# nomic-ai/contrastors

Hardware: AMD Instinct MI355X
Metric: query-doc pairs/sec (whole node), nomic-bert-2048 seq128 global-batch 16384 (higher is better)
Workload: dtype bf16

## Files before the change

contrastors_amd/_C.py:

```python
from __future__ import annotations

import ctypes as C
import os
from pathlib import Path

_PKG = Path(__file__).resolve().parent
LIB_PATH = Path(os.environ.get("CONTRASTORS_HIP_LIB", _PKG / "lib" / "libcontrastors_hip.so"))

CX_OK = 0
_ERR = {-1: "CX_ERR_SHAPE", -2: "CX_ERR_ALIGN", -3: "CX_ERR_ARG", -4: "CX_ERR_LAUNCH"}

vp = C.c_void_p
i32 = C.c_int
i64 = C.c_long
f32 = C.c_float
u64 = C.c_ulonglong
u32 = C.c_uint


class CxLayerWeights(C.Structure):
    _fields_ = (
        [(n, vp) for n in ("Wqkv", "Wout", "Wfc1", "Wfc2", "WqkvT", "WoutT", "Wfc1T", "Wfc2T")]
        + [(n, vp) for n in ("bqkv", "bout", "bfc1", "bfc2")]
        + [(n, vp) for n in ("ln1_g", "ln1_b", "ln2_g", "ln2_b")]
        + [(n, vp) for n in ("gWqkv", "gWout", "gWfc1", "gWfc2")]
        + [(n, vp) for n in ("gbqkv", "gbout", "gbfc1", "gbfc2")]
        + [(n, vp) for n in ("gln1_g", "gln1_b", "gln2_g", "gln2_b")]
    )


class CxEncoderDesc(C.Structure):
    _fields_ = [
        ("n_layer", i32), ("d", i32), ("n_head", i32), ("d_inner", i32), ("gated", i32),
        ("vocab", i32), ("max_pos", i32), ("padding_idx", i32),
        ("ln_eps", f32), ("softmax_scale", f32),
        ("word_emb", vp), ("type_emb", vp), ("pos_emb", vp),
        ("emb_ln_g", vp), ("emb_ln_b", vp),
        ("gword_emb", vp), ("gtype_emb", vp), ("gpos_emb", vp), ("gemb_ln_g", vp), ("gemb_ln_b", vp),
        ("rot_cos", vp), ("rot_sin", vp),
        ("layers", C.POINTER(CxLayerWeights)),
        ("pool_mode", i32), ("normalize", i32),
        ("prenorm", i32),
        ("lnf_g", vp), ("lnf_b", vp), ("glnf_g", vp), ("glnf_b", vp),
        ("Wpatch", vp), ("bpatch", vp), ("cls_token", vp), ("vit_pos", vp),
        ("gWpatch", vp), ("gbpatch", vp), ("gcls_token", vp), ("gvit_pos", vp),
        ("patch_dim", i32),
        ("resid_pdrop", f32), ("embd_pdrop", f32), ("attn_pdrop", f32),
        ("mlp_act", i32), ("lnpre_g", vp), ("lnpre_b", vp), ("glnpre_g", vp), ("glnpre_b", vp),
    ]


class CxChunkBuffers(C.Structure):
    _fields_ = [("T_cap", i64)] + [
        (n, vp)
        for n in (
            "h0", "emb_mean", "emb_rstd", "qkv", "ctx", "lse", "z1", "h1", "mean1", "rstd1", "yg", "act", "z2",
            "h2", "mean2", "rstd2", "pool_norm", "g_a", "g_b", "g_c", "g_wide", "g_act", "tr_a", "tr_b", "delta",
            "ws_f32",
        )
    ] + [("ws_floats", i64)] + [(n, vp) for n in ("zf", "hf", "meanf", "rstdf", "patch_in", "patch_proj")] + [("checkpoint", i32), ("drop_active", i32), ("drop_seed", C.c_ulonglong), ("drop_offset", C.c_ulonglong), ("g_d", vp), ("layer_events", C.POINTER(vp)), ("zpre", vp), ("ckpt_keep", i32), ("patch_keep", vp), ("patch_inv", vp), ("n_keep", i32), ("n_patch_all", i32)]



class CxVitSubLN(C.Structure):
    _fields_ = [(n, vp) for n in ("norm_g", "norm_b", "gnorm_g", "gnorm_b")]


class CxVitExt(C.Structure):
    _fields_ = [("rope_cos", vp), ("rope_sin", vp), ("n_rope", i32), ("n_prefix", i32), ("no_final_ln", i32),
                ("subln_eps", f32), ("sub_ln", C.POINTER(CxVitSubLN)), ("z", vp), ("zmean", vp), ("zrstd", vp),
                ("yg_wide", vp)]


_SIGS = {
    "cx_abi_version": (i32, []),
    "cx_build_info": (C.c_char_p, []),
    "cx_error_string": (C.c_char_p, [i32]),
    "cx_gemm_bf16_nt": (i32, [vp, vp, vp, vp, i32, i32, i32, i32, i32, i32, i32, i32, f32, vp]),
    "cx_gemm_bf16_nt_accum": (i32, [vp, vp, vp, vp, i64, i32, i32, i32, i32, i32, vp]),
    "cx_gemm_bf16_tn_accum": (i32, [vp, vp, vp, vp, i64, i32, i32, i32, i32, i32, vp]),
    "cx_prof_gemm_config": (i32, [i32, i32]),
    "cx_prof_gemm_collect": (i32, [C.POINTER(C.c_double), C.POINTER(C.c_double), C.POINTER(i64), C.POINTER(i64)]),
    "cx_calib_mfma_bf16": (i32, [vp, i32, i32, vp, vp, vp]),
    "cx_calib_copy": (i32, [vp, vp, i64, vp]),
    "cx_transpose_bf16": (i32, [vp, vp, i32, i32, i32, i32, i32, vp]),
    "cx_cast_f32_to_bf16": (i32, [vp, vp, i64, vp]),
    "cx_cast_transpose_f32_to_bf16": (i32, [vp, vp, i32, i32, vp]),
    "cx_cast_transpose_f32_to_bf16_batched": (i32, [vp, i32, i32, vp]),
    "cx_cast_bf16_to_f32": (i32, [vp, vp, i64, vp]),
    "cx_layernorm_fwd": (i32, [vp, vp, vp, vp, vp, vp, vp, vp, i32, i32, f32, vp]),
    "cx_layernorm_bwd": (i32, [vp, vp, vp, vp, vp, vp, vp, vp, vp, vp, vp, i64, i32, i32, vp]),
    "cx_layernorm_bwd_pooled": (i32, [vp, vp, vp, vp, i32, i32, i32, vp, vp, vp, vp, vp, vp, vp, vp, vp, i64, i32, i32, vp]),
    "cx_layernorm_bwd_colsum": (i32, [vp, vp, vp, vp, vp, vp, vp, vp, vp, vp, vp, vp, i64, i32, i32, vp]),
    "cx_dropout_add_layernorm_fwd": (i32, [vp, vp, vp, vp, vp, vp, vp, vp, i32, i32, f32, f32, C.c_ulonglong, C.c_ulonglong,
                                           C.c_uint, vp]),
    "cx_dropout_add_layernorm_bwd": (i32, [vp, vp, vp, vp, vp, vp, vp, vp, vp, vp, vp, i64, i32, i32, f32, C.c_ulonglong,
                                           C.c_ulonglong, C.c_uint, vp]),
    "cx_dropout_add_layernorm_bwd_colsum": (i32, [vp, vp, vp, vp, vp, vp, vp, vp, vp, vp, vp, vp, i64, i32, i32, f32, C.c_ulonglong,
                                                  C.c_ulonglong, C.c_uint, vp]),
    "cx_dropout_scale": (i32, [vp, i64, f32, C.c_ulonglong, C.c_ulonglong, C.c_uint, vp]),
    "cx_layernorm_fwd_mixed": (i32, [vp, vp, vp, vp, vp, vp, vp, vp, i32, i32, f32, i32, vp]),
    "cx_layernorm_bwd_mixed": (i32, [vp, vp, vp, vp, vp, vp, vp, vp, vp, vp, i32, i32, i32, vp]),
    "cx_embed_ln_fwd": (i32, [vp, vp, vp, vp, vp, vp, vp, vp, vp, vp, i32, i32, i32, f32, vp]),
    "cx_embed_ln_bwd": (i32, [vp] * 15 + [i32, i32, i32, i32, vp]),
    "cx_embed_ln_bwd_sorted": (i32, [vp] * 15 + [i32, i32, i32, i32, i32, vp, vp, vp, vp]),
    "cx_swiglu_fwd": (i32, [vp, vp, i32, i32, i32, vp]),
    "cx_swiglu_bwd": (i32, [vp, vp, vp, i32, i32, i32, vp]),
    "cx_gemm_bf16_swiglu": (i32, [vp, vp, vp, vp, i32, i32, i32, i32, i32, i32, i32, vp]),
    "cx_gemm_bf16_nt_residual": (i32, [vp, vp, vp, vp, vp, i32, i32, i32, i32, i32, i32, i32, vp]),
    "cx_gemm_bf16_swiglu_bwd": (i32, [vp, vp, vp, vp, i32, i32, i32, i32, i32, i32, vp]),
    "cx_gemm_bf16_nt_splitk": (i32, [vp, vp, vp, vp, vp, vp, i64, i32, i32, i32, i32, i32, i32, i32, vp]),
    "cx_gemm_bf16_swiglu_gate": (i32, [vp, vp, vp, vp, i32, i32, i32, i32, i32, i32, i32, vp]),
    "cx_gemm_bf16_swiglu_bwd_gate": (i32, [vp, vp, vp, vp, vp, i32, i32, i32, i32, i32, i32, i32, vp]),
    "cx_swiglu_bwd_gate": (i32, [vp, vp, vp, vp, i32, i32, vp]),
    "cx_gemm_bf16_bias_gelu": (i32, [vp, vp, vp, vp, vp, i32, i32, i32, i32, i32, i32, i32, vp]),
    "cx_gemm_bf16_bias_act": (i32, [vp, vp, vp, vp, vp, i32, i32, i32, i32, i32, i32, i32, i32, vp]),
    "cx_bias_gelu_fwd": (i32, [vp, vp, vp, i32, i32, vp]),
    "cx_bias_gelu_bwd": (i32, [vp, vp, vp, vp, i32, i32, vp]),
    "cx_bias_grad": (i32, [vp, vp, i32, i32, i32, vp]),
    "cx_bias_gelu_bwd_colsum": (i32, [vp, vp, vp, vp, vp, i32, i32, vp]),
    "cx_bias_act_fwd": (i32, [vp, vp, vp, i32, i32, i32, vp]),
    "cx_bias_act_bwd_colsum": (i32, [vp, vp, vp, vp, vp, i32, i32, i32, vp]),
    "cx_gemm_bf16_act_bwd": (i32, [vp, vp, vp, vp, vp, vp, i64, i32, i32, i32, i32, i32, i32, i32, i32, vp]),
    "cx_attn_varlen_fwd": (i32, [vp, vp, vp, vp, vp, vp, i32, i32, i32, i32, f32, vp]),
    "cx_attn_varlen_bwd": (i32, [vp] * 9 + [i32, i32, i32, i32, f32, vp]),
    "cx_attn_varlen_bwd_prerotated": (i32, [vp] * 9 + [i32, i32, i32, i32, f32, vp]),
    "cx_attn_varlen_dropout_fwd": (i32, [vp] * 6 + [i32, i32, i32, i32, f32, f32, u64, u64, u32, vp]),
    "cx_attn_varlen_dropout_bwd": (i32, [vp] * 9 + [i32, i32, i32, i32, f32, f32, u64, u64, u32, vp]),
    "cx_ipc_alloc": (i32, [C.POINTER(vp), i64, i32]),
    "cx_ipc_free": (i32, [vp]),
    "cx_ipc_export": (i32, [vp, vp]),
    "cx_ipc_open": (i32, [vp, C.POINTER(vp)]),
    "cx_ipc_close": (i32, [vp]),
    "cx_xgmi_push": (i32, [vp, vp, i64, i64, i32, vp]),
    "cx_xgmi_scatter": (i32, [vp, vp, i32, i64, i32, vp]),
    "cx_xgmi_signal_wait": (i32, [vp, vp, i32, i32, u32, i64, vp, vp]),
    "cx_sum_slots_f32": (i32, [vp, vp, i64, i32, vp]),
    "cx_attn_varlen_kvpacked_fwd": (i32, [vp] * 6 + [i32, i32, i32, i32, i32, f32, vp]),
    "cx_attn_varlen_kvpacked_bwd": (i32, [vp] * 10 + [i32, i32, i32, i32, i32, f32, vp]),
    "cx_rotary_qkv_inplace": (i32, [vp, vp, vp, vp, i32, i32, i32, i32, i32, vp]),
    "cx_rotary_apply": (i32, [vp, i64, vp, vp, vp, i32, i32, i32, i32, i32, vp]),
    "cx_pool_normalize_fwd": (i32, [vp, vp, vp, vp, i32, i32, i32, i32, vp]),
    "cx_pool_normalize_bwd": (i32, [vp, vp, vp, vp, vp, i32, i32, i32, i32, vp]),
    "cx_vit_patchify": (i32, [vp, i32, vp, i32, i32, i32, i32, i32, vp]),
    "cx_vit_assemble_fwd": (i32, [vp, vp, vp, vp, i32, i32, i32, vp]),
    "cx_vit_assemble_bwd": (i32, [vp, vp, vp, vp, i32, i32, i32, vp]),
    "cx_vit_patchify_gather": (i32, [vp, i32, vp, i32, i32, i32, i32, i32, vp, i32, vp]),
    "cx_vit_assemble_fwd_gather": (i32, [vp, vp, vp, vp, i32, i32, i32, vp, vp]),
    "cx_vit_assemble_bwd_gather": (i32, [vp, vp, vp, vp, i32, i32, i32, vp, i32, vp]),
    "cx_vit_forward": (i32, [C.POINTER(CxEncoderDesc), C.POINTER(CxChunkBuffers), vp, i32, vp, i32, i32, i32, i32, i32,
                             i32, vp, vp]),
    "cx_vit_backward": (i32, [C.POINTER(CxEncoderDesc), C.POINTER(CxChunkBuffers), vp, i32, i32, vp, vp, vp]),
    "cx_vit_forward_hidden": (i32, [C.POINTER(CxEncoderDesc), C.POINTER(CxChunkBuffers), vp, i32, vp, i32, i32, i32, i32, i32,
                                    i32, vp, vp]),
    "cx_vit_backward_hidden": (i32, [C.POINTER(CxEncoderDesc), C.POINTER(CxChunkBuffers), vp, i32, i32, vp, vp]),
    "cx_rope2d_qkv_inplace": (i32, [vp, vp, vp, vp, i32, i32, i32, i32, i32, i32, vp]),
    "cx_swiglu_subln_fwd": (i32, [vp, vp, vp, vp, vp, vp, vp, vp, i32, i32, f32, vp]),
    "cx_swiglu_subln_bwd": (i32, [vp] * 11 + [i64, i32, i32, vp]),
    "cx_vit_forward_ex": (i32, [C.POINTER(CxEncoderDesc), C.POINTER(CxChunkBuffers), C.POINTER(CxVitExt), vp, i32, vp, i32, i32,
                                i32, i32, i32, i32, vp, vp]),
    "cx_vit_backward_ex": (i32, [C.POINTER(CxEncoderDesc), C.POINTER(CxChunkBuffers), C.POINTER(CxVitExt), vp, i32, i32, vp, vp,
                                 vp]),
# ... 150 lines not shown
```

contrastors_amd/config.py:

```python
from __future__ import annotations

from typing import Any, Dict, List, Optional, Tuple, Union

import yaml
from pydantic import BaseModel, ConfigDict, model_validator


class TrainArgs(BaseModel):
    model_config = ConfigDict(extra="ignore", validate_assignment=True)
    num_epochs: int = 1
    num_train_steps: Optional[int] = None
    learning_rate: float = 2e-4
    weight_decay: float = 0.01
    eps: Optional[float] = 1e-8
    warmup_steps: Optional[int] = None
    warmup_pct: Optional[float] = None
    cooldown_steps: Optional[int] = None
    checkpoint: Optional[str] = None
    wandb: bool = False
    wandb_project_name: str = ""
    wandb_entity: str = ""
    wandb_run_name: Optional[str] = None
    wandb_group: Optional[str] = None
    log_grads_every: int = 100
    log_lr_every: int = 10
    save_every: Optional[int] = None
    eval_steps: Optional[int] = None
    eval_strategy: Optional[str] = None
    output_dir: Optional[str] = None
    gradient_accumulation_steps: Optional[int] = 1
    schedule_type: str = "cosine"
    max_grad_norm: float = 1.0
    adam_beta1: float = 0.9
    adam_beta2: float = 0.999
    loss_fn: Optional[str] = "clip"
    grad_cache: Optional[bool] = None
    chunk_size: Optional[int] = None
    clamp_logits: Optional[bool] = True
    logit_max: Optional[float] = 100.0
    matryoshka_dims: Optional[List[int]] = None
    matryoshka_loss_weights: Optional[List[float]] = None
    profile: Optional[bool] = False
    use_fp8: Optional[bool] = False
    gradcache_chunk: Union[int, str, None] = "auto"
    gradcache_resident: Union[bool, str, None] = "auto"
    exchange: Optional[str] = "auto"
    exchange_timeout_s: float = 120.0
    overlap_grad_reduce: bool = True
    checkpoint_keep_layers: Union[int, str, None] = "auto"
    distill_loss_fn: str = "mse"
    distill_temperature: float = 1.0

    @model_validator(mode="after")
    def _checks(self):
        from .policy import _parse_chunk, _parse_keep, _parse_resident

        _parse_chunk(self.gradcache_chunk, "train_args.gradcache_chunk")
        _parse_resident(self.gradcache_resident, "train_args.gradcache_resident")
        _parse_keep(self.checkpoint_keep_layers, "train_args.checkpoint_keep_layers")
        if self.distill_loss_fn not in ("mse", "kd", "towers", "stella"):
            raise ValueError(f"Loss function {self.distill_loss_fn} not found in loss function registry")
        if self.exchange not in (None, "auto", "rccl", "oneshot"):
            raise ValueError(f"train_args.exchange must be auto, rccl or oneshot, got {self.exchange!r}")
        if self.use_fp8 and self.matryoshka_dims is not None:
            bad = [d for d in self.matryoshka_dims if d not in (256, 512, 768, 1024)]
            if bad:
                raise ValueError(f"use_fp8 covers similarity widths 256 / 512 / 768 / 1024; matryoshka_dims has {bad}")
        if self.eval_strategy is not None and self.eval_strategy not in ("steps", "epochs"):
            raise ValueError(f"Eval strategy {self.eval_strategy} not found in eval strategy registry")
        if self.eval_strategy == "steps" and self.eval_steps is None:
            raise ValueError("Eval steps must be set if eval strategy is set to steps")
        if self.matryoshka_dims is not None and self.grad_cache:
            raise ValueError("Matryoshka dims cannot be set if grad cache is set")
        return self


class DataArgs(BaseModel):
    model_config = ConfigDict(extra="ignore")
    shuffle: bool = False
    workers: int = 0
    batch_size: int = 16384
    seed: int = 42
    input_shards: Optional[str] = None
    download: Optional[bool] = False
    streaming: Optional[bool] = True
    process_one_shard: Optional[bool] = False
    weighted_sampling: Optional[bool] = False
    verbose: Optional[bool] = False
    sample_negatives: Optional[bool] = False
    query_max_length: Optional[int] = None
    document_max_length: Optional[int] = None
    mlm_prob: Optional[float] = None
    tokenized_dataset: Optional[str] = None
    val_pct: Optional[float] = None
    val_mlm_prob: Optional[float] = None
    mask_on: str = "device"
    task_name: Optional[str] = None
    image_text_shards: Optional[str] = None
# ... 102 lines not shown
```

contrastors_amd/csrc/engine.hip:

```cpp
#include <hip/hip_runtime.h>
#include "../../include/contrastors_hip.h"
#include "ln_workspace.h"

namespace {

#define CX_TRY(expr)              \
    do {                          \
        int rc__ = (expr);        \
        if (rc__ != CX_OK) return rc__; \
    } while (0)

inline long round_up(long v, long m) { return (v + m - 1) / m * m; }

inline int mark_grads_done(const CxChunkBuffers* buf, int idx, void* stream) {
    if (!buf->layer_events || !buf->layer_events[idx]) return CX_OK;
    return hipEventRecord((hipEvent_t)buf->layer_events[idx], (hipStream_t)stream) == hipSuccess ? CX_OK : CX_ERR_LAUNCH;
}

struct Slots {
    const CxChunkBuffers* b;
    const CxEncoderDesc* e;
    long T_cap;
    int d, I, wfc1;
    int mode;
    int first_kept;
    bool kept(int s) const { return mode == 1 || (mode == 2 && s >= first_kept); }
    int sl(int s) const { return mode == 1 ? s : (mode == 2 && s >= first_kept) ? 1 + s - first_kept : 0; }
    int sl_in(int s) const { return mode == 0 ? 0 : s; }
    uint16_t* qkv(int s) const { return b->qkv + (size_t)sl(s) * T_cap * 3 * d; }
    uint16_t* ctx(int s) const { return b->ctx + (size_t)sl(s) * T_cap * d; }
    float* lse(int s) const { return b->lse + (size_t)sl(s) * T_cap * e->n_head; }
    uint16_t* z1(int s) const { return b->z1 + (size_t)(e->prenorm ? sl_in(s) : sl(s)) * T_cap * d; }
    uint16_t* h1(int s) const { return b->h1 + (size_t)sl(s) * T_cap * d; }
    float* mean1(int s) const { return b->mean1 + (size_t)sl(s) * T_cap; }
    float* rstd1(int s) const { return b->rstd1 + (size_t)sl(s) * T_cap; }
    uint16_t* yg(int s) const { return b->yg + (size_t)sl(s) * T_cap * I; }
    uint16_t* act(int s) const { return b->act + (size_t)sl(s) * T_cap * I; }
    uint16_t* z2(int s) const { return b->z2 + (size_t)sl(s) * T_cap * d; }
    uint16_t* h2(int s) const { return b->h2 + (size_t)(e->prenorm ? sl(s) : sl_in(s)) * T_cap * d; }
    float* mean2(int s) const { return b->mean2 + (size_t)sl(s) * T_cap; }
    float* rstd2(int s) const { return b->rstd2 + (size_t)sl(s) * T_cap; }
    uint16_t* ez(const CxVitExt* x, int s) const { return x->z + (size_t)sl(s) * T_cap * I; }
    float* ezmean(const CxVitExt* x, int s) const { return x->zmean + (size_t)sl(s) * T_cap; }
    float* ezrstd(const CxVitExt* x, int s) const { return x->zrstd + (size_t)sl(s) * T_cap; }
};

inline bool ext_rope(const CxVitExt* x) { return x && x->rope_cos; }
inline bool ext_subln(const CxVitExt* x) { return x && x->sub_ln; }
inline bool ext_no_lnf(const CxVitExt* x) { return x && x->no_final_ln; }
int check_ext(const CxVitExt* x, const CxEncoderDesc* e, const CxChunkBuffers* b) {
    if (!x) return CX_OK;
    if (x->rope_cos && (!x->rope_sin || x->n_rope <= 0 || x->n_prefix < 0)) return CX_ERR_ARG;
    if (x->sub_ln) {
        if (!e->gated || !x->z || !x->zmean || !x->zrstd || (!x->yg_wide && !b->g_wide)) return CX_ERR_ARG;
        for (int l = 0; l < e->n_layer; ++l)
            if (!x->sub_ln[l].norm_g || !x->sub_ln[l].norm_b) return CX_ERR_ARG;
    }
    return CX_OK;
}

Slots make_slots(const CxEncoderDesc* enc, const CxChunkBuffers* buf, int save) {
    const int L = enc->n_layer;
    int keep = buf->ckpt_keep < 0 ? 0 : buf->ckpt_keep > L ? L : buf->ckpt_keep;
    return Slots{buf, enc, buf->T_cap, enc->d, enc->d_inner, enc->gated ? 2 * enc->d_inner : enc->d_inner,
                 save ? (buf->checkpoint ? 2 : 1) : 0, L - keep};
}

int check_desc(const CxEncoderDesc* e, const CxChunkBuffers* b, int T) {
    if (!e || !b || !e->layers) return CX_ERR_ARG;
    if (e->n_layer <= 0 || e->d <= 0 || e->n_head <= 0) return CX_ERR_ARG;
    if (e->d != e->n_head * 64) return CX_ERR_SHAPE;
    if ((e->d % 64) != 0 || (e->d_inner % 64) != 0) return CX_ERR_SHAPE;
    if (b->T_cap < round_up(T, 64)) return CX_ERR_SHAPE;
    return CX_OK;
}

int wgrad_split(int out_f, int in_f, long Tp) {
    const long tiles = (long)((out_f + 127) / 128) * ((in_f + 127) / 128);
    const long nk = Tp / 64;
    long s = (512 + tiles - 1) / tiles;
    if (s > nk / 2) s = nk / 2;
    if (s < 1) s = 1;
    return (int)s;
}

int wgrad(const uint16_t* dY, int out_f, const uint16_t* X, int in_f, float* gW, const CxChunkBuffers* b, int T,
          void* stream) {
    if (!gW) return CX_OK;
    const int rc = cx_gemm_bf16_tn_accum(dY, X, gW, b->ws_f32, b->ws_floats, T, out_f, in_f, out_f, in_f, stream);
    if (rc != CX_ERR_SHAPE) return rc;
    if (!b->tr_a || !b->tr_b) return CX_ERR_ARG;
    const int Tp = (int)round_up(T, 64);
    CX_TRY(cx_transpose_bf16(dY, b->tr_a, T, out_f, out_f, Tp, Tp, stream));
    CX_TRY(cx_transpose_bf16(X, b->tr_b, T, in_f, in_f, Tp, Tp, stream));
    return cx_gemm_bf16_nt_accum(b->tr_a, b->tr_b, gW, b->ws_f32, b->ws_floats, out_f, in_f, Tp, Tp, Tp, stream);
}

int proj_residual(const uint16_t* x, const uint16_t* W, const float* bias, const uint16_t* residual, uint16_t* out, int T,
                  int N, int K, bool* folded, void* stream, const CxChunkBuffers* buf = nullptr) {
    *folded = false;
    if (buf && buf->ws_f32 && (long)((T + 255) / 256) * ((N + 255) / 256) <= 64 && K >= 1536) {
        const int rc = cx_gemm_bf16_nt_splitk(x, W, out, bias, residual, buf->ws_f32, buf->ws_floats, T, N, K, K, K, N, N, stream);
        if (rc != CX_ERR_SHAPE) {
            *folded = residual != nullptr && rc == CX_OK;
            return rc;
        }
    }
    if (residual) {
        const int rc = cx_gemm_bf16_nt_residual(x, W, out, bias, residual, T, N, K, K, K, N, N, stream);
        if (rc != CX_ERR_SHAPE) {
            *folded = rc == CX_OK;
            return rc;
        }
    }
    return cx_gemm_bf16_nt(x, W, out, bias, T, N, K, K, K, N, 0, 1, 1.f, stream);
}

bool gelu_fused_shape(int T, int N, int K) {
    return T > 0 && (K % 64) == 0 && (N % 8) == 0;
}

struct BlockRunner {
    const CxEncoderDesc* enc;
    const CxChunkBuffers* buf;
    const Slots& s;
    const int32_t* cu_seqlens;
    int Bc, T, max_seqlen;
    void* stream;
    const CxVitExt* ext = nullptr;

    int mlp_up(const CxLayerWeights& w, const uint16_t* x, int l, bool keep) const {
        const int d = enc->d, I = enc->d_inner;
        if (ext_subln(ext)) {
            uint16_t* yg = ext->yg_wide ? ext->yg_wide : buf->g_wide;
            CX_TRY(cx_gemm_bf16_nt(x, w.Wfc1, yg, w.bfc1, T, 2 * I, d, d, d, 2 * I, 0, 1, 1.f, stream));
            const CxVitSubLN& n = ext->sub_ln[l];
            return cx_swiglu_subln_fwd(yg, n.norm_g, n.norm_b, keep ? s.yg(l) : nullptr, s.act(l), s.ez(ext, l), s.ezmean(ext, l),
                                       s.ezrstd(ext, l), T, I, ext->subln_eps, stream);
        }
        if (enc->gated) {
            return cx_gemm_bf16_swiglu_gate(x, w.Wfc1, keep ? s.yg(l) : nullptr, s.act(l), T, I, d, d, d, I, I, stream);
        }
        const int rc = cx_gemm_bf16_bias_act(x, w.Wfc1, w.bfc1, keep ? s.yg(l) : nullptr, s.act(l), T, s.wfc1, d, d, d, s.wfc1,
                                             I, enc->mlp_act, stream);
        if (rc != CX_ERR_SHAPE) return rc;
        CX_TRY(cx_gemm_bf16_nt(x, w.Wfc1, s.yg(l), nullptr, T, s.wfc1, d, d, d, s.wfc1, 0, 1, 1.f, stream));
        return cx_bias_act_fwd(s.yg(l), w.bfc1, s.act(l), T, I, enc->mlp_act, stream);
    }
    int mlp(const CxLayerWeights& w, const uint16_t* x, int l, uint16_t* out, const uint16_t* residual, bool keep,
            bool* folded) const {
        CX_TRY(mlp_up(w, x, l, keep));
        return proj_residual(ext_subln(ext) ? s.ez(ext, l) : s.act(l), w.Wfc2, w.bfc2, residual, out, T, enc->d, enc->d_inner, folded, stream, buf);
    }
    int attn(const CxLayerWeights& w, const uint16_t* x, int l, uint16_t* out, const uint16_t* residual, bool* folded) const {
        const int d = enc->d;
        CX_TRY(cx_gemm_bf16_nt(x, w.Wqkv, s.qkv(l), w.bqkv, T, 3 * d, d, d, d, 3 * d, 0, 1, 1.f, stream));
        if (ext_rope(ext))
            CX_TRY(cx_rope2d_qkv_inplace(s.qkv(l), cu_seqlens, ext->rope_cos, ext->rope_sin, ext->n_rope, Bc, enc->n_head, T,
                                         ext->n_prefix, 1, stream));
        if (buf->drop_active && enc->attn_pdrop > 0.f) {
            CX_TRY(cx_attn_varlen_dropout_fwd(s.qkv(l), cu_seqlens, enc->rot_cos, enc->rot_sin, s.ctx(l), s.lse(l), Bc,
                                              enc->n_head, T, max_seqlen, enc->softmax_scale, enc->attn_pdrop, buf->drop_seed,
                                              buf->drop_offset, (unsigned)(2 * enc->n_layer + 1 + l), stream));
        } else if (enc->rot_cos && max_seqlen > 128) {
            CX_TRY(cx_rotary_qkv_inplace(s.qkv(l), cu_seqlens, enc->rot_cos, enc->rot_sin, Bc, enc->n_head, T, max_seqlen, 1,
                                         stream));
            CX_TRY(cx_attn_varlen_fwd(s.qkv(l), cu_seqlens, nullptr, nullptr, s.ctx(l), s.lse(l), Bc, enc->n_head, T, max_seqlen,
                                      enc->softmax_scale, stream));
        } else {
            CX_TRY(cx_attn_varlen_fwd(s.qkv(l), cu_seqlens, enc->rot_cos, enc->rot_sin, s.ctx(l), s.lse(l), Bc, enc->n_head, T,
                                      max_seqlen, enc->softmax_scale, stream));
        }
        return proj_residual(s.ctx(l), w.Wout, w.bout, residual, out, T, d, d, folded, stream);
    }
    int post_block(int l, const uint16_t* h_in, bool keep) const {
        const CxLayerWeights& w = enc->layers[l];
        const int d = enc->d;
        bool f1 = false, f2 = false;
        if (drop()) {
            const float p = enc->resid_pdrop;
            CX_TRY(attn(w, h_in, l, s.z1(l), nullptr, &f1));
            CX_TRY(cx_dropout_add_layernorm_fwd(s.z1(l), h_in, w.ln1_g, w.ln1_b, s.h1(l), keep ? s.z1(l) : nullptr, s.mean1(l),
                                                s.rstd1(l), T, d, enc->ln_eps, p, buf->drop_seed, buf->drop_offset, 2 * l, stream));
            CX_TRY(mlp(w, s.h1(l), l, s.z2(l), nullptr, keep, &f2));
            return cx_dropout_add_layernorm_fwd(s.z2(l), s.h1(l), w.ln2_g, w.ln2_b, s.h2(l), keep ? s.z2(l) : nullptr, s.mean2(l),
                                                s.rstd2(l), T, d, enc->ln_eps, p, buf->drop_seed, buf->drop_offset, 2 * l + 1,
                                                stream);
        }
        CX_TRY(attn(w, h_in, l, s.z1(l), h_in, &f1));
        CX_TRY(cx_layernorm_fwd(s.z1(l), f1 ? nullptr : h_in, w.ln1_g, w.ln1_b, s.h1(l), (keep && !f1) ? s.z1(l) : nullptr,
                                s.mean1(l), s.rstd1(l), T, d, enc->ln_eps, stream));
        CX_TRY(mlp(w, s.h1(l), l, s.z2(l), s.h1(l), keep, &f2));
        return cx_layernorm_fwd(s.z2(l), f2 ? nullptr : s.h1(l), w.ln2_g, w.ln2_b, s.h2(l), (keep && !f2) ? s.z2(l) : nullptr,
                                s.mean2(l), s.rstd2(l), T, d, enc->ln_eps, stream);
    }
    bool drop() const { return buf->drop_active && enc->resid_pdrop > 0.f; }
    int pre_block(int l, const uint16_t* x, const uint16_t* r, bool r_folded, bool keep, bool up_only, const uint16_t** x_out,
                  const uint16_t** r_out, bool* folded_out) const {
        const CxLayerWeights& w = enc->layers[l];
        const int d = enc->d, L = enc->n_layer;
        CX_TRY(cx_layernorm_fwd(x, r, w.ln1_g, w.ln1_b, s.h1(l), (r_folded && x == s.z1(l)) ? nullptr : s.z1(l), s.mean1(l),
                                s.rstd1(l), T, d, enc->ln_eps, stream));
        bool f1 = false, f2 = false;
        CX_TRY(attn(w, s.h1(l), l, s.z2(l), s.z1(l), &f1));
        CX_TRY(cx_layernorm_fwd(s.z2(l), f1 ? nullptr : s.z1(l), w.ln2_g, w.ln2_b, s.h2(l), f1 ? nullptr : s.z2(l), s.mean2(l),
                                s.rstd2(l), T, d, enc->ln_eps, stream));
        if (up_only) return mlp_up(w, s.h2(l), l, keep);
        uint16_t* nxt = (l + 1 < L) ? s.z1(l + 1) : buf->zf;
        CX_TRY(mlp(w, s.h2(l), l, nxt, s.z2(l), keep, &f2));
        *x_out = nxt;
        *r_out = f2 ? nullptr : s.z2(l);
        *folded_out = f2;
        return CX_OK;
    }
};

int blocks_forward(const CxEncoderDesc* enc, const CxChunkBuffers* buf, const Slots& s, const uint16_t* h0,
                   const int32_t* cu_seqlens, int Bc, int T, int max_seqlen, int save, const uint16_t** h_final,
                   void* stream, const CxVitExt* ext = nullptr) {
    const int d = enc->d, L = enc->n_layer;
    const BlockRunner run{enc, buf, s, cu_seqlens, Bc, T, max_seqlen, stream, ext};
    if (!enc->prenorm) {
        const uint16_t* h_in = h0;
        for (int l = 0; l < L; ++l) {
            CX_TRY(run.post_block(l, h_in, save != 0 && s.kept(l)));
            h_in = s.h2(l);
        }
        *h_final = h_in;
        return CX_OK;
    }
    if (!buf->zf || !buf->hf || !buf->meanf || !buf->rstdf || (!ext_no_lnf(ext) && (!enc->lnf_g || !enc->lnf_b))) return CX_ERR_ARG;
    if (buf->drop_active && enc->resid_pdrop > 0.f) return CX_ERR_ARG;
    const uint16_t* x = h0;
    const uint16_t* r = nullptr;
    bool r_folded = false;
    for (int l = 0; l < L; ++l) {
        CX_TRY(run.pre_block(l, x, r, r_folded, save != 0 && s.kept(l), false, &x, &r, &r_folded));
        if (save == 2 && !r_folded) return CX_ERR_SHAPE;
    }
    if (ext_no_lnf(ext)) {
        if (!r_folded || x != buf->zf) return CX_ERR_SHAPE;
        *h_final = buf->zf;
        return CX_OK;
    }
    CX_TRY(cx_layernorm_fwd(x, r, enc->lnf_g, enc->lnf_b, buf->hf, r_folded ? nullptr : buf->zf, buf->meanf, buf->rstdf, T,
// ... 533 lines not shown
```

contrastors_amd/csrc/gemm_api.hip:

```cpp
#include "cx_common.h"
#include "../../include/contrastors_hip.h"
#include "gemm_params.h"
#include <mutex>

namespace {

constexpr int BK = 64;

__global__ __launch_bounds__(256) void splitk_reduce_kernel(const float* __restrict__ part, float* __restrict__ out, long n4,
                                                            long slab, int splits) {
    const long stride = (long)gridDim.x * blockDim.x;
    for (long i = (long)blockIdx.x * blockDim.x + threadIdx.x; i < n4; i += stride) {
        float4 a = reinterpret_cast<const float4*>(out)[i];
        for (int s = 0; s < splits; ++s) {
            const float4 v = reinterpret_cast<const float4*>(part + s * slab)[i];
            a.x += v.x; a.y += v.y; a.z += v.z; a.w += v.w;
        }
        reinterpret_cast<float4*>(out)[i] = a;
    }
}

int reduce_slabs(const float* ws, float* out, long slab, int split, hipStream_t s) {
    const long n4 = slab / 4;
    long g = (n4 + 255) / 256;
// ... 113 lines not shown
    const int Tp = (T + BK - 1) / BK * BK;
    GemmParams p = base_params(dY, A, ws, nullptr, O, I, Tp, ld_dy, ld_a, I);
    const long tiles = (long)(O / 256) * (I / 256), nk = Tp / BK;
    long max_split = nk / 4;
    if (max_split > ws_floats / slab) max_split = ws_floats / slab;
    if (max_split > 32) max_split = 32;
    p.split_k = (int)choose_split(tiles, max_split);
    {
        ProfScope prof(2.0 * (double)T * (double)O * (double)I, (hipStream_t)stream);
        if (cx_launch_gemm_v6_tn(p, (hipStream_t)stream) != hipSuccess) return CX_ERR_LAUNCH;
    }
    return reduce_slabs(ws, G, slab, p.split_k, (hipStream_t)stream);
}

int cx_gemm_bf16_swiglu(const uint16_t* X, const uint16_t* W, uint16_t* YG, uint16_t* Act, int M, int I, int K, int ldx,
                        int ldw, int ld_yg, int ld_act, void* stream) {
    if (M <= 0 || I <= 0) return CX_OK;
    if (K <= 0 || (K % BK) != 0 || (I % 32) != 0) return CX_ERR_SHAPE;
    if ((ldx % 8) != 0 || (ldw % 8) != 0 || (ld_yg % 4) != 0 || (ld_act % 4) != 0) return CX_ERR_ALIGN;
    if (!Act) return CX_ERR_ARG;
    GemmParams p = base_params(X, W, YG, nullptr, M, 2 * I, K, ldx, ldw, ld_yg);
    p.Out2 = Act; p.ldo2 = ld_act;
    ProfScope prof(2.0 * (double)M * (double)(2 * I) * (double)K, (hipStream_t)stream);
    const hipError_t e = ((ld_yg % 8) == 0 && (ld_act % 8) == 0)
                             ? cx_launch_gemm_v6(p, GEMM_EPI_SWIGLU, (hipStream_t)stream)
                             : cx_launch_gemm_v5(p, 0, GEMM_OUT_BF16, GEMM_EPI_SWIGLU, (hipStream_t)stream);
    return e == hipSuccess ? CX_OK : CX_ERR_LAUNCH;
}

int cx_gemm_bf16_swiglu_gate(const uint16_t* X, const uint16_t* W, uint16_t* G, uint16_t* Act, int M, int I, int K, int ldx,
                             int ldw, int ld_g, int ld_act, void* stream) {
    if (M <= 0 || I <= 0) return CX_OK;
    if (K <= 0 || (K % BK) != 0 || (I % 32) != 0 || (ld_g % 8) != 0 || (ld_act % 8) != 0) return CX_ERR_SHAPE;
    if ((ldx % 8) != 0 || (ldw % 8) != 0) return CX_ERR_ALIGN;
    if (!Act) return CX_ERR_ARG;
    GemmParams p = base_params(X, W, G, nullptr, M, 2 * I, K, ldx, ldw, ld_g);
    p.Out2 = Act; p.ldo2 = ld_act;
    ProfScope prof(2.0 * (double)M * (double)(2 * I) * (double)K, (hipStream_t)stream);
    return cx_launch_gemm_v6(p, GEMM_EPI_SWIGLU_G, (hipStream_t)stream) == hipSuccess ? CX_OK : CX_ERR_LAUNCH;
}

int cx_gemm_bf16_nt_residual(const uint16_t* X, const uint16_t* W, uint16_t* Out, const float* bias, const uint16_t* Residual,
                             int M, int N, int K, int ldx, int ldw, int ldo, int ldr, void* stream) {
    if (M <= 0 || N <= 0) return CX_OK;
    if (!Residual || !Out) return CX_ERR_ARG;
    if (K <= 0 || (K % 64) != 0 || (N % 8) != 0 || (ldo % 8) != 0 || (ldr % 8) != 0) return CX_ERR_SHAPE;
    if ((ldx % 8) != 0 || (ldw % 8) != 0) return CX_ERR_ALIGN;
    GemmParams p = base_params(X, W, Out, bias, M, N, K, ldx, ldw, ldo);
    p.Out2 = const_cast<uint16_t*>(Residual); p.ldo2 = ldr;
    ProfScope prof(2.0 * (double)M * (double)N * (double)K, (hipStream_t)stream);
    return cx_launch_gemm_v6(p, GEMM_EPI_NONE, (hipStream_t)stream) == hipSuccess ? CX_OK : CX_ERR_LAUNCH;
}

int cx_gemm_bf16_bias_gelu(const uint16_t* X, const uint16_t* W, const float* bias, uint16_t* Pre, uint16_t* Act, int M, int N,
                           int K, int ldx, int ldw, int ld_pre, int ld_act, void* stream) {
    return cx_gemm_bf16_bias_act(X, W, bias, Pre, Act, M, N, K, ldx, ldw, ld_pre, ld_act, 0, stream);
}

int cx_gemm_bf16_bias_act(const uint16_t* X, const uint16_t* W, const float* bias, uint16_t* Pre, uint16_t* Act, int M, int N,
                          int K, int ldx, int ldw, int ld_pre, int ld_act, int act, void* stream) {
    if (M <= 0 || N <= 0) return CX_OK;
    if (!Act || (act != 0 && act != 1)) return CX_ERR_ARG;
    if (K <= 0 || (K % 64) != 0 || (N % 8) != 0 || (ld_act % 8) != 0 || (Pre && (ld_pre % 8) != 0)) return CX_ERR_SHAPE;
    if ((ldx % 8) != 0 || (ldw % 8) != 0) return CX_ERR_ALIGN;
    GemmParams p = base_params(X, W, Pre, bias, M, N, K, ldx, ldw, ld_pre);
    p.Out2 = Act; p.ldo2 = ld_act;
    p.act = act;
    ProfScope prof(2.0 * (double)M * (double)N * (double)K, (hipStream_t)stream);
    return cx_launch_gemm_v6(p, act == 1 ? GEMM_EPI_QGELU : GEMM_EPI_GELU, (hipStream_t)stream) == hipSuccess ? CX_OK : CX_ERR_LAUNCH;
}

int cx_gemm_bf16_swiglu_bwd(const uint16_t* dY, const uint16_t* W, const uint16_t* YG, uint16_t* dYG, int M, int I, int K,
                            int ldx, int ldw, int ld_yg, void* stream) {
    if (M <= 0 || I <= 0) return CX_OK;
    if (!dY || !W || !YG || !dYG) return CX_ERR_ARG;
    if (K <= 0 || (K % 64) != 0 || (I % 256) != 0 || (ld_yg % 8) != 0 || ld_yg < 2 * I) return CX_ERR_SHAPE;
    if ((ldx % 8) != 0 || (ldw % 8) != 0) return CX_ERR_ALIGN;
    GemmParams p = base_params(dY, W, dYG, nullptr, M, I, K, ldx, ldw, ld_yg);
    p.Out2 = const_cast<uint16_t*>(YG); p.ldo2 = ld_yg;
    ProfScope prof(2.0 * (double)M * (double)I * (double)K, (hipStream_t)stream);
    return cx_launch_gemm_v6(p, GEMM_EPI_SWIGLU_BWD, (hipStream_t)stream) == hipSuccess ? CX_OK : CX_ERR_LAUNCH;
}

int cx_gemm_bf16_swiglu_bwd_gate(const uint16_t* dY, const uint16_t* W, const uint16_t* Act, const uint16_t* G, uint16_t* dYG,
                                 int M, int I, int K, int ldx, int ldw, int ld_ag, int ld_dyg, void* stream) {
    if (M <= 0 || I <= 0) return CX_OK;
    if (!dY || !W || !Act || !G || !dYG) return CX_ERR_ARG;
    if (K <= 0 || (K % 64) != 0 || (I % 256) != 0 || (ld_dyg % 8) != 0 || ld_dyg < 2 * I || (ld_ag % 8) != 0 || ld_ag < I)
        return CX_ERR_SHAPE;
    if ((ldx % 8) != 0 || (ldw % 8) != 0) return CX_ERR_ALIGN;
    GemmParams p = base_params(dY, W, dYG, nullptr, M, I, K, ldx, ldw, ld_dyg);
    p.Out2 = const_cast<uint16_t*>(Act); p.ldo2 = ld_ag;
    p.In3 = G;
    ProfScope prof(2.0 * (double)M * (double)I * (double)K, (hipStream_t)stream);
    return cx_launch_gemm_v6(p, GEMM_EPI_SWIGLU_BWD_AG, (hipStream_t)stream) == hipSuccess ? CX_OK : CX_ERR_LAUNCH;
}

int cx_gemm_bf16_act_bwd(const uint16_t* dY, const uint16_t* W, const uint16_t* Pre, uint16_t* dPre, float* dbias, float* ws,
                         long ws_floats, int M, int N, int K, int ldx, int ldw, int ld_pre, int ld_dpre, int act, void* stream) {
    if (M <= 0 || N <= 0) return CX_OK;
    if (!dY || !W || !Pre || !dPre || (act != 0 && act != 1)) return CX_ERR_ARG;
    if (K <= 0 || (K % 64) != 0 || (N % 8) != 0 || (ld_pre % 8) != 0 || (ld_dpre % 8) != 0) return CX_ERR_SHAPE;
    if ((ldx % 8) != 0 || (ldw % 8) != 0) return CX_ERR_ALIGN;
    const int nblocks = (M + 127) / 128;
    if (dbias && (!ws || ws_floats < (long)nblocks * N)) return CX_ERR_SHAPE;
    GemmParams p = base_params(dY, W, dPre, nullptr, M, N, K, ldx, ldw, ld_dpre);
// ... 41 lines not shown
```

contrastors_amd/csrc/gemm_bf16.hip:

```cpp
#include "cx_common.h"
#include "../../include/contrastors_hip.h"
#include "gemm_params.h"

namespace {

constexpr int BM = 128, BN = 128, BK = 64;
constexpr int TILE_BYTES = 128 * BK * 2;

typedef __attribute__((address_space(3))) void* lds_void_ptr;
typedef const __attribute__((address_space(1))) void* glb_void_ptr;

enum OutMode { OUT_BF16 = GEMM_OUT_BF16, OUT_F32 = GEMM_OUT_F32, OUT_F32_ATOMIC = GEMM_OUT_F32_ATOMIC };

struct StageRegs { uint4 r0, r1, r2, r3; };

CX_DEVICE uint4 stage_load(const bf16_t* __restrict__ base, int ld, int row0, int nrows, int k0, int tid, int p) {
    const int r = p * 32 + (tid >> 3);
    int gr = row0 + r;
    gr = gr < nrows ? gr : nrows - 1;
    return *reinterpret_cast<const uint4*>(base + (size_t)gr * ld + k0 + (tid & 7) * 8);
}

template <bool GLDS>
CX_DEVICE void stage_tile(const bf16_t* __restrict__ base, int ld, int row0, int nrows, int k0, char* lds_tile,
// ... 745 lines not shown
    p.tiles_m = p.tiles_n = 0; p.split_k = 1; p.alpha = 1.f; p.dbg = g_dbg;
    p.Out2 = Act; p.ldo2 = ld_act; p.sup_m = p.sup_n = 0;
    int slot = -1;
    if (g_prof.enabled) {
        if ((g_prof.launches % g_prof.stride) == 0 && g_prof.used < GemmProf::CAP) {
            slot = g_prof.used++;
            if (slot >= g_prof.created) {
                if (hipEventCreate(&g_prof.ev0[slot]) != hipSuccess || hipEventCreate(&g_prof.ev1[slot]) != hipSuccess)
                    return CX_ERR_LAUNCH;
                g_prof.created = slot + 1;
            }
            g_prof.flop[slot] = 2.0 * (double)M * (double)(2 * I) * (double)K;
            (void)hipEventRecord(g_prof.ev0[slot], (hipStream_t)stream);
        }
        ++g_prof.launches;
    }
    hipError_t e = cx_launch_gemm_v5(p, 0, GEMM_OUT_BF16, GEMM_EPI_SWIGLU, (hipStream_t)stream);
    if (slot >= 0) (void)hipEventRecord(g_prof.ev1[slot], (hipStream_t)stream);
    return e == hipSuccess ? CX_OK : CX_ERR_LAUNCH;
}

int cx_gemm_bf16_nt_residual(const uint16_t* X, const uint16_t* W, uint16_t* Out, const float* bias,
                             const uint16_t* Residual, int M, int N, int K, int ldx, int ldw, int ldo, int ldr,
                             void* stream) {
    if (M <= 0 || N <= 0) return CX_OK;
    if (!Residual || !Out) return CX_ERR_ARG;
    if (K <= 0 || (K % 64) != 0 || (N % 8) != 0 || (ldo % 8) != 0 || (ldr % 8) != 0) return CX_ERR_SHAPE;
    if ((ldx % 8) != 0 || (ldw % 8) != 0) return CX_ERR_ALIGN;
    if (cx_gemm_get_variant() != 6) return CX_ERR_SHAPE;
    GemmParams p;
    p.X = X; p.W = W; p.Out = Out; p.bias = bias;
    p.M = M; p.N = N; p.K = K; p.ldx = ldx; p.ldw = ldw; p.ldo = ldo;
    p.tiles_m = p.tiles_n = 0; p.split_k = 1; p.alpha = 1.f; p.dbg = g_dbg;
    p.Out2 = const_cast<uint16_t*>(Residual); p.ldo2 = ldr; p.sup_m = p.sup_n = 0; p.trace = nullptr;
    int slot = -1;
    if (g_prof.enabled) {
        if ((g_prof.launches % g_prof.stride) == 0 && g_prof.used < GemmProf::CAP) {
            slot = g_prof.used++;
            if (slot >= g_prof.created) {
                if (hipEventCreate(&g_prof.ev0[slot]) != hipSuccess || hipEventCreate(&g_prof.ev1[slot]) != hipSuccess)
                    return CX_ERR_LAUNCH;
                g_prof.created = slot + 1;
            }
            g_prof.flop[slot] = 2.0 * (double)M * (double)N * (double)K;
            (void)hipEventRecord(g_prof.ev0[slot], (hipStream_t)stream);
        }
        ++g_prof.launches;
    }
    const hipError_t e = cx_launch_gemm_v6(p, GEMM_EPI_NONE, (hipStream_t)stream);
    if (slot >= 0) (void)hipEventRecord(g_prof.ev1[slot], (hipStream_t)stream);
    return e == hipSuccess ? CX_OK : CX_ERR_LAUNCH;
}

int cx_gemm_bf16_bias_gelu(const uint16_t* X, const uint16_t* W, const float* bias, uint16_t* Pre, uint16_t* Act, int M,
                           int N, int K, int ldx, int ldw, int ld_pre, int ld_act, void* stream) {
    return cx_gemm_bf16_bias_act(X, W, bias, Pre, Act, M, N, K, ldx, ldw, ld_pre, ld_act, 0, stream);
}

int cx_gemm_bf16_bias_act(const uint16_t* X, const uint16_t* W, const float* bias, uint16_t* Pre, uint16_t* Act, int M,
                          int N, int K, int ldx, int ldw, int ld_pre, int ld_act, int act, void* stream) {
    if (M <= 0 || N <= 0) return CX_OK;
    if (!Act || (act != 0 && act != 1)) return CX_ERR_ARG;
    if (K <= 0 || (K % 64) != 0 || (N % 8) != 0 || (ld_act % 8) != 0 || (Pre && (ld_pre % 8) != 0)) return CX_ERR_SHAPE;
    if ((ldx % 8) != 0 || (ldw % 8) != 0) return CX_ERR_ALIGN;
    if (cx_gemm_get_variant() != 6) return CX_ERR_SHAPE;
    GemmParams p;
    p.X = X; p.W = W; p.Out = Pre; p.bias = bias;
    p.M = M; p.N = N; p.K = K; p.ldx = ldx; p.ldw = ldw; p.ldo = ld_pre;
    p.tiles_m = p.tiles_n = 0; p.split_k = 1; p.alpha = 1.f; p.dbg = g_dbg;
    p.Out2 = Act; p.ldo2 = ld_act; p.sup_m = p.sup_n = 0; p.trace = nullptr;
    p.act = act;
    int slot = -1;
    if (g_prof.enabled) {
        if ((g_prof.launches % g_prof.stride) == 0 && g_prof.used < GemmProf::CAP) {
            slot = g_prof.used++;
            if (slot >= g_prof.created) {
                if (hipEventCreate(&g_prof.ev0[slot]) != hipSuccess || hipEventCreate(&g_prof.ev1[slot]) != hipSuccess)
                    return CX_ERR_LAUNCH;
                g_prof.created = slot + 1;
            }
            g_prof.flop[slot] = 2.0 * (double)M * (double)N * (double)K;
            (void)hipEventRecord(g_prof.ev0[slot], (hipStream_t)stream);
        }
        ++g_prof.launches;
    }
    const hipError_t e = cx_launch_gemm_v6(p, act == 1 ? GEMM_EPI_QGELU : GEMM_EPI_GELU, (hipStream_t)stream);
    if (slot >= 0) (void)hipEventRecord(g_prof.ev1[slot], (hipStream_t)stream);
    return e == hipSuccess ? CX_OK : CX_ERR_LAUNCH;
}

int cx_gemm_bf16_swiglu_bwd(const uint16_t* dY, const uint16_t* W, const uint16_t* YG, uint16_t* dYG, int M, int I, int K,
                            int ldx, int ldw, int ld_yg, void* stream) {
    if (M <= 0 || I <= 0) return CX_OK;
    if (!dY || !W || !YG || !dYG) return CX_ERR_ARG;
    if (K <= 0 || (K % 64) != 0 || (I % 256) != 0 || (ld_yg % 8) != 0 || ld_yg < 2 * I) return CX_ERR_SHAPE;
    if ((ldx % 8) != 0 || (ldw % 8) != 0) return CX_ERR_ALIGN;
    if (cx_gemm_get_variant() != 6) return CX_ERR_SHAPE;
    GemmParams p;
    p.X = dY; p.W = W; p.Out = dYG; p.bias = nullptr;
    p.M = M; p.N = I; p.K = K; p.ldx = ldx; p.ldw = ldw; p.ldo = ld_yg;
    p.tiles_m = p.tiles_n = 0; p.split_k = 1; p.alpha = 1.f; p.dbg = g_dbg;
    p.Out2 = const_cast<uint16_t*>(YG); p.ldo2 = ld_yg; p.sup_m = p.sup_n = 0; p.trace = nullptr;
    int slot = -1;
    if (g_prof.enabled) {
        if ((g_prof.launches % g_prof.stride) == 0 && g_prof.used < GemmProf::CAP) {
            slot = g_prof.used++;
// ... 92 lines not shown
```

contrastors_amd/csrc/gemm_bf16_v6.hip:

```cpp
#include "cx_common.h"
#include "../../include/contrastors_hip.h"
#include "gemm_params.h"
#include <type_traits>

namespace {

#ifndef CX_V6_HI_EARLY
#define CX_V6_HI_EARLY 1
#endif
#ifndef CX_V6_OPAQUE
#define CX_V6_OPAQUE 1
#endif
#ifndef CX_V6_NT
#define CX_V6_NT 3
#endif
template <int J>
__device__ __forceinline__ void v6_dma_m0(uint32_t slot_base) {
    asm volatile("s_add_u32 m0, %0, %1" ::"s"(slot_base), "n"(J * 4096) : "memory", "scc");
}
__device__ __forceinline__ void v6_dma_ld(uint32_t off, const bf16_t* base) {
    asm volatile("global_load_lds_dwordx4 %0, %1" ::"v"(off), "s"(base) : "memory");
}
template <int J>
__device__ __forceinline__ void v6_dma_full(uint32_t slot_base, uint32_t off, const bf16_t* base) {
    asm volatile("s_add_u32 m0, %0, %1\n\ts_nop 0\n\tglobal_load_lds_dwordx4 %2, %3" ::"s"(slot_base), "n"(J * 4096), "v"(off),
                 "s"(base) : "memory", "scc");
}
typedef unsigned int cx_u32x4 __attribute__((ext_vector_type(4)));
__device__ __forceinline__ void gst_nt(void* ptr, uint4 v) {
    cx_u32x4 t = {v.x, v.y, v.z, v.w};
    __builtin_nontemporal_store(t, reinterpret_cast<cx_u32x4*>(ptr));
}
__device__ __forceinline__ uint4 gld_nt(const void* ptr) {
    const cx_u32x4 t = __builtin_nontemporal_load(reinterpret_cast<const cx_u32x4*>(ptr));
    return make_uint4(t.x, t.y, t.z, t.w);
}
#if CX_V6_NT & 1
#define gst(ptr, v) gst_nt((ptr), (v))
#else
#define gst(ptr, v) (*reinterpret_cast<uint4*>(ptr) = (v))
#endif
#if CX_V6_NT & 2
#define gld(ptr) gld_nt(ptr)
#else
#define gld(ptr) (*reinterpret_cast<const uint4*>(ptr))
#endif

typedef __attribute__((address_space(3))) void* lds_void_ptr;
typedef const __attribute__((address_space(1))) void* glb_void_ptr;

constexpr int BM6 = 256, BN6 = 256, BK6 = 64;
constexpr int XS6 = 32768;
constexpr int LDS6 = 5 * XS6;

struct Frags6 {
// ... 201 lines not shown
        const char* xs = dsm + xs_slot * XS6;
        const char* ws = dsm + (3 + ws_slot) * XS6;
        const int nxs_slot = xs_slot == 2 ? 0 : xs_slot + 1, nws_slot = ws_slot ^ 1;
        if constexpr (decltype(first)::value) {
            CX_SEG(mma1z, F0, 0, 64, F1, xs, ws, 1, RS_ == 2 ? 0 : 1, RS_, 1, RS_ == 2 ? 1 : 17, DS_, 0, 8);
        } else {
            CX_SEG(mma1, F0, 0, 64, F1, xs, ws, 1, RS_ == 2 ? 0 : 1, RS_, 1, RS_ == 2 ? 1 : 17, DS_, 0, 8);
        }
        w_advance();
        CX_SEG(mma1, F1, 0, 32, F0, xs, ws, 0, 0, 0, 2, 0, RS_ == 2 ? 8 : DS_, 0, 4);
        asm volatile("s_waitcnt lgkmcnt(0)" ::: "memory");
        if constexpr ((DBG & 128) != 0) {
            const long long w0_ = (long long)__builtin_amdgcn_s_memtime();
            asm volatile("s_waitcnt vmcnt(4)" ::: "memory");
            const long long w1_ = (long long)__builtin_amdgcn_s_memtime();
            ph[decltype(first)::value ? 0 : 1] += w1_ - w0_;
        } else if constexpr ((DBG & 32) == 0) {
            asm volatile("s_waitcnt vmcnt(4)" ::: "memory");
        }
        if constexpr ((DBG & 2) == 0) __builtin_amdgcn_s_barrier();
        const char* nxs = dsm + nxs_slot * XS6;
        const char* nws = dsm + (3 + nws_slot) * XS6;
        CX_SEG(mma1, F1, 32, 64, F0, nxs, nws, 0, RS_ == 2 ? 32 : 33, RS_, 2, RS_ == 2 ? 33 : 49, RS_ == 2 ? 8 : DS_, 4, 4);
        x_advance();
        if constexpr ((DBG & 128) != 0 && decltype(first)::value) {
            const long long now_ = (long long)__builtin_amdgcn_s_memtime();
            kt0_cyc += now_ - t_last;
        }
        ++cp_kt;
        pxs_slot = xs_slot;
        pws_slot = ws_slot;
        xs_slot = nxs_slot;
        ws_slot = nws_slot;
    };

#pragma unroll 1
    while (cp_tile >= 0) {
        cp_kt = 0;
        kt_body(std::true_type{});
#pragma unroll 1
        while (cp_kt < nk) kt_body(std::false_type{});

        {
            CX_PH(2);
            asm volatile("s_nop 7\n\ts_nop 7\n\ts_nop 7" ::: "memory");
            const int tn = cp_tile & 255, tm = cp_tile >> 8;
            const int m0 = tm * BM6 + wm * 128, n0 = tn * BN6 + wn * 128;
            char* my = ((wave < 2) ? dsm + pxs_slot * XS6 : dsm + (3 + pws_slot) * XS6) + (wave & 1) * 16384;
            constexpr int ROWB = 272;
            auto prow = [&](int q) { return (q >> 1) * 16 + l15; };
            auto pcol = [&](int q) { return (q & 1) * 16 + 4 * g4; };
            auto qoff = [](int q, int rowb) { return (q >> 1) * 16 * rowb + (q & 1) * 32; };
            if constexpr ((DBG & 16) != 0) {
            } else if constexpr (EPI == GEMM_EPI_NONE || EPI == GEMM_EPI_ACT_BWD || EPI == GEMM_EPI_QACT_BWD) {
                constexpr bool ACTB = EPI == GEMM_EPI_ACT_BWD || EPI == GEMM_EPI_QACT_BWD;
                float cs0 = 0.f, cs1 = 0.f, cs2 = 0.f, cs3 = 0.f, cs4 = 0.f, cs5 = 0.f, cs6 = 0.f, cs7 = 0.f;
                constexpr int act_kind = EPI == GEMM_EPI_QACT_BWD ? CX_ACT_QUICK_GELU : CX_ACT_GELU;
                auto mul_grad = [&](uint4& v, const uint4& r) {
#define CX_MG(w_, ca, cb)                                                                              \
    {                                                                                                 \
        const float o0 = bf16lo_to_f32(v.w_) * act_grad(bf16lo_to_f32(r.w_), act_kind);               \
        const float o1 = bf16hi_to_f32(v.w_) * act_grad(bf16hi_to_f32(r.w_), act_kind);               \
        v.w_ = pack_bf16x2(o0, o1);                                                                   \
        ca += bf16lo_to_f32(v.w_);                                                                    \
        cb += bf16hi_to_f32(v.w_);                                                                    \
    }
                    CX_MG(x, cs0, cs1) CX_MG(y, cs2, cs3) CX_MG(z, cs4, cs5) CX_MG(w, cs6, cs7)
#undef CX_MG
                };
                auto flush_colsum = [&]() {
                    if constexpr (ACTB) {
                        float c[8] = {cs0, cs1, cs2, cs3, cs4, cs5, cs6, cs7};
#pragma unroll
                        for (int e = 0; e < 8; ++e) {
                            c[e] += __shfl_xor(c[e], 16, 64);
                            c[e] += __shfl_xor(c[e], 32, 64);
                        }
                        const int n = n0 + (lane & 15) * 8;
                        if (p.colsum_part && lane < 16 && m0 < p.M && n + 8 <= p.N) {
                            float* dst = p.colsum_part + (size_t)(m0 >> 7) * p.N + n;
                            *reinterpret_cast<float4*>(dst) = make_float4(c[0], c[1], c[2], c[3]);
                            *reinterpret_cast<float4*>(dst + 4) = make_float4(c[4], c[5], c[6], c[7]);
                        }
                    }
                };
                const bool add_bias = p.bias != nullptr;
                const bf16_t* resid = reinterpret_cast<const bf16_t*>(p.Out2);
                auto fast_tile = [&](auto with_resid) {
                    constexpr bool RES = decltype(with_resid)::value;
                    const int rrow = lane >> 4, rch = lane & 15;
                    bf16_t* outp = reinterpret_cast<bf16_t*>(p.Out) + (size_t)(m0 + rrow) * p.ldo + n0 + rch * 8;
                    const bf16_t* resp = RES ? resid + (size_t)(m0 + rrow) * p.ldo2 + n0 + rch * 8 : nullptr;
                    const char* rd = my + rrow * ROWB + rch * 16;
                    char* wr = my + prow(0) * ROWB + pcol(0) * 2;
                    uint2 pk[16];
                    auto pack_pass = [&](int b) {
#pragma unroll
                        for (int a = 0; a < 4; ++a) {
                            float blk[16];
                            v6_read_block(4 * b + a, blk);
#pragma unroll
                            for (int q = 0; q < 4; ++q) {
                                pk[a * 4 + q].x = pack_bf16x2(blk[4 * q], blk[4 * q + 1]);
                                pk[a * 4 + q].y = pack_bf16x2(blk[4 * q + 2], blk[4 * q + 3]);
                            }
                        }
                    };
                    auto stage = [&]() {
#pragma unroll
                        for (int a = 0; a < 4; ++a)
#pragma unroll
                            for (int q = 0; q < 4; ++q) *reinterpret_cast<uint2*>(wr + a * 64 + qoff(q, ROWB)) = pk[a * 4 + q];
                    };
                    uint4 r0 = {}, r1 = {}, r2 = {}, r3 = {}, r4 = {}, r5 = {}, r6 = {}, r7 = {};
#define CX_RES_ROWS(b_)                                                                                   \
    r0 = gld(resp + (size_t)((b_) * 32 + 0) * p.ldo2);                          \
    r1 = gld(resp + (size_t)((b_) * 32 + 4) * p.ldo2);                          \
    r2 = gld(resp + (size_t)((b_) * 32 + 8) * p.ldo2);                          \
    r3 = gld(resp + (size_t)((b_) * 32 + 12) * p.ldo2);                         \
    r4 = gld(resp + (size_t)((b_) * 32 + 16) * p.ldo2);                         \
    r5 = gld(resp + (size_t)((b_) * 32 + 20) * p.ldo2);                         \
    r6 = gld(resp + (size_t)((b_) * 32 + 24) * p.ldo2);                         \
    r7 = gld(resp + (size_t)((b_) * 32 + 28) * p.ldo2);
                    auto add_res = [&](uint4& v, const uint4& r) {
                        v.x = pack_bf16x2(bf16lo_to_f32(v.x) + bf16lo_to_f32(r.x), bf16hi_to_f32(v.x) + bf16hi_to_f32(r.x));
                        v.y = pack_bf16x2(bf16lo_to_f32(v.y) + bf16lo_to_f32(r.y), bf16hi_to_f32(v.y) + bf16hi_to_f32(r.y));
                        v.z = pack_bf16x2(bf16lo_to_f32(v.z) + bf16lo_to_f32(r.z), bf16hi_to_f32(v.z) + bf16hi_to_f32(r.z));
                        v.w = pack_bf16x2(bf16lo_to_f32(v.w) + bf16lo_to_f32(r.w), bf16hi_to_f32(v.w) + bf16hi_to_f32(r.w));
                    };
                    auto one_pass = [&](auto bc) {
                        constexpr int b = decltype(bc)::value;
                        uint4 v0 = *reinterpret_cast<const uint4*>(rd + 0 * ROWB), v1 = *reinterpret_cast<const uint4*>(rd + 4 * ROWB),
                              v2 = *reinterpret_cast<const uint4*>(rd + 8 * ROWB), v3 = *reinterpret_cast<const uint4*>(rd + 12 * ROWB),
                              v4 = *reinterpret_cast<const uint4*>(rd + 16 * ROWB), v5 = *reinterpret_cast<const uint4*>(rd + 20 * ROWB),
                              v6 = *reinterpret_cast<const uint4*>(rd + 24 * ROWB), v7 = *reinterpret_cast<const uint4*>(rd + 28 * ROWB);
                        __builtin_amdgcn_sched_barrier(0);
                        if constexpr (b < 3) pack_pass(b + 1);
                        __builtin_amdgcn_sched_barrier(0);
                        if constexpr (RES) {
                            add_res(v0, r0); add_res(v1, r1); add_res(v2, r2); add_res(v3, r3);
                            add_res(v4, r4); add_res(v5, r5); add_res(v6, r6); add_res(v7, r7);
                            if constexpr (b < 3) {
                                __builtin_amdgcn_sched_barrier(0);
                                CX_RES_ROWS(b + 1)
                                __builtin_amdgcn_sched_barrier(0);
                            }
                        }
                        if constexpr (b < 3) stage();
                        bf16_t* o = outp + (size_t)(b * 32) * p.ldo;
                        if constexpr ((DBG & 64) != 0) {
                            const uint4 vs[8] = {v0, v1, v2, v3, v4, v5, v6, v7};
#pragma unroll
                            for (int i = 0; i < 8; ++i) asm volatile("" ::"v"(vs[i].x), "v"(vs[i].y), "v"(vs[i].z), "v"(vs[i].w));
                            asm volatile("" ::"v"(o));
                            return;
                        }
                        gst(o, v0);
                        gst(o + (size_t)4 * p.ldo, v1);
                        gst(o + (size_t)8 * p.ldo, v2);
                        gst(o + (size_t)12 * p.ldo, v3);
                        gst(o + (size_t)16 * p.ldo, v4);
                        gst(o + (size_t)20 * p.ldo, v5);
                        gst(o + (size_t)24 * p.ldo, v6);
                        gst(o + (size_t)28 * p.ldo, v7);
                    };
                    if constexpr (RES) { CX_RES_ROWS(0) }
                    pack_pass(0);
                    stage();
                    one_pass(std::integral_constant<int, 0>{});
                    one_pass(std::integral_constant<int, 1>{});
                    one_pass(std::integral_constant<int, 2>{});
                    one_pass(std::integral_constant<int, 3>{});
#undef CX_RES_ROWS
                };
                auto fast_tile_actb = [&]() {
                    const int rrow = lane >> 4, rch = lane & 15;
                    bf16_t* outp = reinterpret_cast<bf16_t*>(p.Out) + (size_t)(m0 + rrow) * p.ldo + n0 + rch * 8;
                    const bf16_t* resp = resid + (size_t)(m0 + rrow) * p.ldo2 + n0 + rch * 8;
                    const char* rd = my + rrow * ROWB + rch * 16;
                    char* wr = my + prow(0) * ROWB + pcol(0) * 2;
                    auto stage_pass = [&](int b) {
#pragma unroll
                        for (int a = 0; a < 4; ++a) {
                            float blk[16];
                            v6_read_block(4 * b + a, blk);
#pragma unroll
                            for (int q = 0; q < 4; ++q) {
                                uint2 pk2;
                                pk2.x = pack_bf16x2(blk[4 * q], blk[4 * q + 1]);
                                pk2.y = pack_bf16x2(blk[4 * q + 2], blk[4 * q + 3]);
                                *reinterpret_cast<uint2*>(wr + a * 64 + qoff(q, ROWB)) = pk2;
                            }
                            __builtin_amdgcn_sched_barrier(0);
                        }
                    };
                    uint4 r0, r1, r2, r3;
#define CX_PRE_ROWS(hh_)                                                        \
    r0 = gld(resp + (size_t)((hh_) * 16 + 0) * p.ldo2);                         \
    r1 = gld(resp + (size_t)((hh_) * 16 + 4) * p.ldo2);                         \
    r2 = gld(resp + (size_t)((hh_) * 16 + 8) * p.ldo2);                         \
    r3 = gld(resp + (size_t)((hh_) * 16 + 12) * p.ldo2);
                    auto half_pass = [&](auto hc) {
                        constexpr int hh = decltype(hc)::value;
                        constexpr int h = hh & 1;
                        uint4 v0 = *reinterpret_cast<const uint4*>(rd + (h * 16 + 0) * ROWB), v1 = *reinterpret_cast<const uint4*>(rd + (h * 16 + 4) * ROWB),
                              v2 = *reinterpret_cast<const uint4*>(rd + (h * 16 + 8) * ROWB), v3 = *reinterpret_cast<const uint4*>(rd + (h * 16 + 12) * ROWB);
                        __builtin_amdgcn_sched_barrier(0);
                        mul_grad(v0, r0); __builtin_amdgcn_sched_barrier(0);
                        mul_grad(v1, r1); __builtin_amdgcn_sched_barrier(0);
                        mul_grad(v2, r2); __builtin_amdgcn_sched_barrier(0);
                        mul_grad(v3, r3); __builtin_amdgcn_sched_barrier(0);
                        if constexpr (hh < 7) { CX_PRE_ROWS(hh + 1) }
                        __builtin_amdgcn_sched_barrier(0);
                        bf16_t* o = outp + (size_t)(hh * 16) * p.ldo;
                        gst(o, v0);
                        gst(o + (size_t)4 * p.ldo, v1);
                        gst(o + (size_t)8 * p.ldo, v2);
// ... 25 lines not shown
                            CX_RES_LOAD(0, r0) CX_RES_LOAD(1, r1) CX_RES_LOAD(2, r2) CX_RES_LOAD(3, r3)
                            CX_RES_LOAD(4, r4) CX_RES_LOAD(5, r5) CX_RES_LOAD(6, r6) CX_RES_LOAD(7, r7)
#undef CX_RES_LOAD
                        }
#pragma unroll
                        for (int a = 0; a < 4; ++a) {
                            float blk[16];
                            v6_read_block(4 * b + a, blk);
#pragma unroll
                            for (int q = 0; q < 4; ++q) {
                                const int nl = a * 32 + pcol(q);
                                float v[4];
#pragma unroll
                                for (int e = 0; e < 4; ++e) v[e] = blk[4 * q + e];
                                if constexpr (!decltype(plain)::value) {
#pragma unroll
                                    for (int e = 0; e < 4; ++e) v[e] *= p.alpha;
                                    if (add_bias) {
                                        const int n = n0 + nl;
                                        if (n < p.N) {
                                            const float4 bv = *reinterpret_cast<const float4*>(p.bias + n);
                                            v[0] += bv.x; v[1] += bv.y; v[2] += bv.z; v[3] += bv.w;
                                        }
                                    }
                                }
                                uint2 pk;
                                pk.x = pack_bf16x2(v[0], v[1]);
                                pk.y = pack_bf16x2(v[2], v[3]);
                                *reinterpret_cast<uint2*>(my + prow(q) * ROWB + nl * 2) = pk;
                            }
                        }
#pragma unroll
                        for (int ps = 0; ps < 8; ++ps) {
                            const int row = ps * 4 + (lane >> 4), ch = lane & 15;
                            const int m = m0 + b * 32 + row, n = n0 + ch * 8;
                            uint4 vv = *reinterpret_cast<const uint4*>(my + row * ROWB + ch * 16);
                            if (resid && ACTB) {
                                const uint4 rr = ps == 0 ? r0 : ps == 1 ? r1 : ps == 2 ? r2 : ps == 3 ? r3 : ps == 4 ? r4 : ps == 5 ? r5
                                                 : ps == 6 ? r6 : r7;
                                if (m < p.M && n + 8 <= p.N) mul_grad(vv, rr);
                            } else if (resid) {
                                const uint4 rr = ps == 0 ? r0 : ps == 1 ? r1 : ps == 2 ? r2 : ps == 3 ? r3 : ps == 4 ? r4 : ps == 5 ? r5
                                                 : ps == 6 ? r6 : r7;
                                vv.x = pack_bf16x2(bf16lo_to_f32(vv.x) + bf16lo_to_f32(rr.x), bf16hi_to_f32(vv.x) + bf16hi_to_f32(rr.x));
                                vv.y = pack_bf16x2(bf16lo_to_f32(vv.y) + bf16lo_to_f32(rr.y), bf16hi_to_f32(vv.y) + bf16hi_to_f32(rr.y));
                                vv.z = pack_bf16x2(bf16lo_to_f32(vv.z) + bf16lo_to_f32(rr.z), bf16hi_to_f32(vv.z) + bf16hi_to_f32(rr.z));
                                vv.w = pack_bf16x2(bf16lo_to_f32(vv.w) + bf16lo_to_f32(rr.w), bf16hi_to_f32(vv.w) + bf16hi_to_f32(rr.w));
                            }
                            if (m < p.M && n + 8 <= p.N)
                                gst(reinterpret_cast<bf16_t*>(p.Out) + (size_t)m * p.ldo + n, vv);
                        }
                    }
                };
                if constexpr (ACTB) {
                    if (fast) {
                        fast_tile_actb();
                    } else {
                        store_tile(std::true_type{});
                    }
                    flush_colsum();
                } else if (fast) {
                    if (resid) {
                        fast_tile(std::true_type{});
                    } else {
                        fast_tile(std::false_type{});
                    }
                } else if (p.alpha == 1.f && !add_bias) {
                    store_tile(std::true_type{});
                } else {
                    store_tile(std::false_type{});
                }
            } else if constexpr (IS_SWIGLU_BWD) {
                const bf16_t* yg_in = reinterpret_cast<const bf16_t*>(p.Out2);
                const bf16_t* g_in = reinterpret_cast<const bf16_t*>(p.In3);
                bf16_t* dyg = reinterpret_cast<bf16_t*>(p.Out);
                const int c0 = 2 * n0;
                auto bwd_elem = [&](float yv, float gv, float dv, float& dyo, float& dgo) {
                    if constexpr (AG) {
                        swiglu_bwd_from_act(dv, yv, gv, dyo, dgo);
                    } else {
                        const float sg = __builtin_amdgcn_rcpf(1.f + __builtin_amdgcn_exp2f(-1.4426950408889634f * gv));
                        const float gs = gv * sg;
                        dyo = gs * dv;
                        dgo = (sg + gs * (1.f - sg)) * dv * yv;
                    }
                };
                auto bwd_quad = [&](const float (&yv)[4], const float (&gv)[4], const float* dv, float (&dyo)[4], float (&dgo)[4]) {
                    if constexpr (AG) {
#pragma unroll
                        for (int h = 0; h < 2; ++h) {
                            cx_f2 y2, g2;
                            swiglu_bwd_from_act2(cx_f2{dv[2 * h], dv[2 * h + 1]}, cx_f2{yv[2 * h], yv[2 * h + 1]},
                                                 cx_f2{gv[2 * h], gv[2 * h + 1]}, y2, g2);
                            dyo[2 * h] = y2.x; dyo[2 * h + 1] = y2.y;
                            dgo[2 * h] = g2.x; dgo[2 * h + 1] = g2.y;
                        }
                    } else {
#pragma unroll
                        for (int e = 0; e < 4; ++e) bwd_elem(yv[e], gv[e], dv[e], dyo[e], dgo[e]);
                    }
                };
                auto cell = [&](int row, int colbyte) { return my + row * 512 + ((((colbyte >> 4) ^ row) & 31) << 4) + (colbyte & 15); };
                const bool fast_bwd = m0 + 128 <= p.M && n0 + 128 <= p.N;
                if (fast_bwd) {
                    int lane_e = lane;
#if CX_V6_OPAQUE >= 1
                    asm volatile("" : "+v"(lane_e));
#endif
                    const int lrow = lane_e >> 5, lch = lane_e & 31;
                    const bf16_t* src = AG ? ((lch & 4) ? g_in : yg_in) + (size_t)(m0 + lrow) * p.ldo2 + n0 + (lch >> 3) * 32 + (lch & 3) * 8
                                           : yg_in + (size_t)(m0 + lrow) * p.ldo2 + c0 + lch * 8;
                    bf16_t* dst = dyg + (size_t)(m0 + lrow) * p.ldo + c0 + lch * 8;
                    uint4 t0, t1, t2, t3, t4, t5, t6, t7, t8, t9, t10, t11, t12, t13, t14, t15;
#define CX_L(i, b_) t##i = gld(src + (size_t)((b_) * 32 + (i) * 2) * p.ldo2);
#define CX_LOAD_LO(b_) CX_L(0, b_) CX_L(1, b_) CX_L(2, b_) CX_L(3, b_) CX_L(4, b_) CX_L(5, b_) CX_L(6, b_) CX_L(7, b_)
#define CX_LOAD_HI(b_) CX_L(8, b_) CX_L(9, b_) CX_L(10, b_) CX_L(11, b_) CX_L(12, b_) CX_L(13, b_) CX_L(14, b_) CX_L(15, b_)
#define CX_S(i) *reinterpret_cast<uint4*>(cell((i) * 2 + lrow, lch * 16)) = t##i;
#define CX_STAGE_ALL CX_S(0) CX_S(1) CX_S(2) CX_S(3) CX_S(4) CX_S(5) CX_S(6) CX_S(7) CX_S(8) CX_S(9) CX_S(10) CX_S(11) CX_S(12) CX_S(13) CX_S(14) CX_S(15)
// ... 642 lines not shown
    w_advance(1);
    issue_x_tile();
    x_advance(2);
    asm volatile("s_waitcnt vmcnt(8)" ::: "memory");
    __builtin_amdgcn_s_barrier();
#pragma unroll
    for (int i = 0; i < 16; ++i) read_one(F0, 0, 0, 0, i);

    int xs_slot = 0, ws_slot = 0;
    auto kt_body = [&](auto first, int t) {
        constexpr int RS_ = CX_V6_RD_SPREAD, DS_ = CX_V6_DMA_SPREAD;
        const int nxs_slot = xs_slot == 2 ? 0 : xs_slot + 1, nws_slot = ws_slot ^ 1;
        if constexpr (decltype(first)::value) {
            CX_SEG(mma1z, F0, 0, 64, F1, xs_slot, ws_slot, 1, RS_ == 2 ? 0 : 1, RS_, 1, RS_ == 2 ? 1 : 17, DS_, 0, 8);
        } else {
            CX_SEG(mma1, F0, 0, 64, F1, xs_slot, ws_slot, 1, RS_ == 2 ? 0 : 1, RS_, 1, RS_ == 2 ? 1 : 17, DS_, 0, 8);
        }
        w_advance(t + 2);
        CX_SEG(mma1, F1, 0, 32, F0, xs_slot, ws_slot, 0, 0, 0, 2, 0, RS_ == 2 ? 8 : DS_, 0, 4);
        asm volatile("s_waitcnt lgkmcnt(0)" ::: "memory");
        asm volatile("s_waitcnt vmcnt(4)" ::: "memory");
        __builtin_amdgcn_s_barrier();
        CX_SEG(mma1, F1, 32, 64, F0, nxs_slot, nws_slot, 0, RS_ == 2 ? 32 : 33, RS_, 2, RS_ == 2 ? 33 : 49, RS_ == 2 ? 8 : DS_, 4, 4);
        x_advance(t + 3);
        xs_slot = nxs_slot;
        ws_slot = nws_slot;
    };
    kt_body(std::true_type{}, 0);
#pragma unroll 1
    for (int t = 1; t < nk; ++t) kt_body(std::false_type{}, t);
#undef CX_SEG
#undef CX_DMA_M0
#undef CX_DMA_LD

    asm volatile("s_waitcnt vmcnt(0)\n\ts_nop 7\n\ts_nop 7\n\ts_nop 7" ::: "memory");
    float* part = reinterpret_cast<float*>(p.Out) + (size_t)sk * p.M * p.ldo;
#pragma unroll
    for (int b = 0; b < 4; ++b) {
        float* rowp = part + (size_t)(m0 + wm * 128 + b * 32 + l15) * p.ldo + n0 + wn * 128 + 4 * g4;
        float* rowq = rowp + (size_t)16 * p.ldo;
#pragma unroll
        for (int a = 0; a < 4; ++a) v6_store_block_f32(4 * b + a, rowp + a * 32, rowq + a * 32);
    }
}

#ifndef CX_V7_POLICY
#define CX_V7_POLICY 1
#endif
#ifndef CX_PRODUCT
int g_v7_mode = -1;
#else
constexpr int g_v7_mode = -1;
#endif
bool v7_takes(const GemmParams& p, int epi) {
    const int mode = g_v7_mode >= 0 ? (g_v7_mode ? 2 : 0) : CX_V7_POLICY;
    if (mode == 0 || !cx_gemm_v7_covers(p, epi)) return false;
    if (mode == 2) return true;
    if (epi == GEMM_EPI_SWIGLU_G) return false;
    const long tiles256 = (long)((p.M + BM6 - 1) / BM6) * ((p.N + BN6 - 1) / BN6);
    return tiles256 <= 400;
}

#ifndef CX_PRODUCT
int g_v6_dbg = 0;
long long* g_v6_trace = nullptr;
int g_v6_force_gn = 0;
#else
constexpr int g_v6_force_gn = 0;
#endif

int cx_gemm_v6_groups(int tiles_m, int tiles_n, int K) {
    if (g_v6_force_gn) return g_v6_force_gn;
    const double xb = (double)tiles_m * 256 * K * 2, wb = (double)tiles_n * 256 * K * 2;
    int best = 1;
    double best_cost = 0;
    for (int gn = 1; gn <= 8; gn *= 2) {
        const int gm = 8 / gn;
        if ((tiles_n % gn) != 0 || (tiles_m % gm) != 0) continue;
        const double slice = wb / gn;
        const double rounds = (double)tiles_m / gm * (tiles_n / gn) / 32.0;
        const double wcost = slice <= 2.5 * 1048576 ? gm * wb : (rounds < 1 ? 1 : rounds) * slice * 8;
        const double cost = gn * xb + wcost;
        if (gn == 1 || cost < best_cost) { best = gn; best_cost = cost; }
    }
    return best;
}

}

#ifndef CX_PRODUCT
void cx_gemm_v6_set_trace(long long* buf) { g_v6_trace = buf; }
void cx_gemm_v6_set_ablate(int mask) { g_v6_dbg = mask; }
void cx_gemm_v6_force_groups(int gn) { g_v6_force_gn = (gn == 1 || gn == 2 || gn == 4 || gn == 8) ? gn : 0; }
void cx_gemm_v7_set_mode(int mode) { g_v7_mode = mode < 0 ? -1 : (mode ? 1 : 0); }
#endif

hipError_t cx_launch_gemm_v6_tn(GemmParams p, hipStream_t stream) {
    static CxLdsOptIn lds;
    if (!lds.ensure(reinterpret_cast<const void*>(&gemm_bf16_v6tn_kernel), LDS6)) return hipErrorInvalidValue;
    p.tiles_m = p.M / BM6;
    p.tiles_n = p.N / BN6;
    hipLaunchKernelGGL(gemm_bf16_v6tn_kernel, dim3(p.tiles_m * p.tiles_n * p.split_k), dim3(256), LDS6, stream, p);
    return hipGetLastError();
}

namespace {
__global__ __launch_bounds__(256) void colsum_part_reduce_kernel(const float* __restrict__ part, float* dst, int nblocks, int N) {
    __shared__ float red[4][64];
    const int col = blockIdx.x * 64 + (threadIdx.x & 63), grp = threadIdx.x >> 6;
    float sacc = 0.f;
    if (col < N) {
#pragma unroll 4
        for (int b = grp; b < nblocks; b += 4) sacc += part[(size_t)b * N + col];
    }
    red[grp][threadIdx.x & 63] = sacc;
    __syncthreads();
    if (grp == 0 && col < N) dst[col] += (red[0][threadIdx.x] + red[1][threadIdx.x]) + (red[2][threadIdx.x] + red[3][threadIdx.x]);
}
}
hipError_t cx_launch_colsum_part_reduce(const float* part, float* dst, int nblocks, int N, hipStream_t stream) {
    hipLaunchKernelGGL(colsum_part_reduce_kernel, dim3((N + 63) / 64), dim3(256), 0, stream, part, dst, nblocks, N);
    return hipGetLastError();
}

hipError_t cx_launch_gemm_v6(GemmParams p, int epi, hipStream_t stream) {
    if (v7_takes(p, epi)) return cx_launch_gemm_v7(p, epi, g_v6_force_gn, stream);
    p.tiles_m = (p.M + BM6 - 1) / BM6;
    p.tiles_n = (p.N + BN6 - 1) / BN6;
    if (p.tiles_n > 256) return hipErrorInvalidValue;
    p.sup_n = cx_gemm_v6_groups(p.tiles_m, p.tiles_n, p.K);
#ifndef CX_PRODUCT
    if (epi == GEMM_EPI_NONE && g_v6_dbg) {
        p.trace = g_v6_trace;
        switch (g_v6_dbg) {
            case 1: return launch6<GEMM_EPI_NONE, 1>(p, stream);
            case 2: return launch6<GEMM_EPI_NONE, 2>(p, stream);
            case 4: return launch6<GEMM_EPI_NONE, 4>(p, stream);
            case 16: return launch6<GEMM_EPI_NONE, 16>(p, stream);
            case 32: return launch6<GEMM_EPI_NONE, 32>(p, stream);
            case 33: return launch6<GEMM_EPI_NONE, 33>(p, stream);
            case 35: return launch6<GEMM_EPI_NONE, 35>(p, stream);
            case 39: return launch6<GEMM_EPI_NONE, 39>(p, stream);
            case 55: return launch6<GEMM_EPI_NONE, 55>(p, stream);
            case 59: return launch6<GEMM_EPI_NONE, 59>(p, stream);
            case 64: return launch6<GEMM_EPI_NONE, 64>(p, stream);
            case 128: return launch6<GEMM_EPI_NONE, 128>(p, stream);
            default: break;
        }
    }
#endif
#ifndef CX_PRODUCT
    if (g_v6_dbg == 128 && (epi == GEMM_EPI_SWIGLU_G || epi == GEMM_EPI_SWIGLU || epi == GEMM_EPI_SWIGLU_BWD_AG)) {
        p.trace = g_v6_trace;
        return epi == GEMM_EPI_SWIGLU_G ? launch6<GEMM_EPI_SWIGLU_G, 128>(p, stream)
               : epi == GEMM_EPI_SWIGLU ? launch6<GEMM_EPI_SWIGLU, 128>(p, stream) : launch6<GEMM_EPI_SWIGLU_BWD_AG, 128>(p, stream);
    }
#endif
    return epi == GEMM_EPI_SWIGLU ? launch6<GEMM_EPI_SWIGLU>(p, stream)
           : epi == GEMM_EPI_SWIGLU_G ? launch6<GEMM_EPI_SWIGLU_G>(p, stream)
           : epi == GEMM_EPI_SWIGLU_BWD_AG ? launch6<GEMM_EPI_SWIGLU_BWD_AG>(p, stream)
           : epi == GEMM_EPI_GELU ? launch6<GEMM_EPI_GELU>(p, stream)
           : epi == GEMM_EPI_QGELU ? launch6<GEMM_EPI_QGELU>(p, stream)
           : epi == GEMM_EPI_SWIGLU_BWD ? launch6<GEMM_EPI_SWIGLU_BWD>(p, stream)
           : epi == GEMM_EPI_ACT_BWD ? (p.act == CX_ACT_QUICK_GELU ? launch6<GEMM_EPI_QACT_BWD>(p, stream) : launch6<GEMM_EPI_ACT_BWD>(p, stream))
                                  : launch6<GEMM_EPI_NONE>(p, stream);
}
```

contrastors_amd/csrc/gemm_params.h:

```cpp
#pragma once
#include <hip/hip_runtime.h>
#include <stdint.h>

enum { GEMM_OUT_BF16 = 0, GEMM_OUT_F32 = 1, GEMM_OUT_F32_ATOMIC = 2, GEMM_OUT_F32_PARTIAL = 3 };
enum { GEMM_EPI_NONE = 0, GEMM_EPI_SWIGLU = 1, GEMM_EPI_GELU = 2, GEMM_EPI_SWIGLU_BWD = 3,
       GEMM_EPI_QGELU = 4,
       GEMM_EPI_SWIGLU_G = 5,
       GEMM_EPI_SWIGLU_BWD_AG = 6,
       GEMM_EPI_QACT_BWD = 8,
       GEMM_EPI_ACT_BWD = 7 };

struct GemmParams {
    const uint16_t* X;
    const uint16_t* W;
    void* Out;
    const float* bias;
    int M, N, K;
    int ldx, ldw, ldo;
    int tiles_m, tiles_n, split_k;
    float alpha;
    int dbg;
    int act;
    void* Out2;
    int ldo2;
    const uint16_t* In3;
    float* colsum_part;
    int sup_m, sup_n;
    long long* trace;
};

hipError_t cx_launch_gemm_v5(GemmParams p, int form, int out_mode, int epi, hipStream_t stream);
hipError_t cx_launch_gemm_v6(GemmParams p, int epi, hipStream_t stream);
void cx_gemm_v6_force_groups(int gn);
void cx_gemm_v6_set_trace(long long* buf);
void cx_gemm_v6_set_ablate(int mask);
hipError_t cx_launch_gemm_v6_tn(GemmParams p, hipStream_t stream);
hipError_t cx_launch_colsum_part_reduce(const float* part, float* dst, int nblocks, int N, hipStream_t stream);
bool cx_gemm_v7_covers(const GemmParams& p, int epi);
hipError_t cx_launch_gemm_v7(GemmParams p, int epi, int force_gn, hipStream_t stream);
void cx_gemm_v7_set_trace(long long* buf);
int cx_gemm_v7_occupancy_query(void);
void cx_gemm_v7_set_ablate(int mask);
void cx_gemm_v7_set_flags(int f);
void cx_gemm_v7_set_period(int cycles);
void cx_gemm_v7_set_mode(int mode);
void cx_gemm_v5_set_persistent(bool on);
void cx_gemm_v5_set_use_v6(bool on);
bool cx_gemm_v5_get_use_v6(void);
void cx_gemm_v5_set_trace(long long* buf);
```

contrastors_amd/csrc/layernorm.hip:

```cpp
#include "cx_common.h"
#include "ln_workspace.h"
#include "../../include/contrastors_hip.h"

namespace {

CX_DEVICE void unpack4_bf16(const uint2 u, float (&v)[4]) {
    v[0] = bf16lo_to_f32(u.x); v[1] = bf16hi_to_f32(u.x);
    v[2] = bf16lo_to_f32(u.y); v[3] = bf16hi_to_f32(u.y);
}
CX_DEVICE void load4_bf16(const bf16_t* p, float (&v)[4]) { unpack4_bf16(*reinterpret_cast<const uint2*>(p), v); }
CX_DEVICE uint2 store4_bf16(bf16_t* p, const float (&v)[4]) {
    uint2 u;
    u.x = pack_bf16x2(v[0], v[1]);
    u.y = pack_bf16x2(v[2], v[3]);
    *reinterpret_cast<uint2*>(p) = u;
    return u;
}
CX_DEVICE void load4_f32(const float* p, float (&v)[4]) {
    const float4 u = *reinterpret_cast<const float4*>(p);
    v[0] = u.x; v[1] = u.y; v[2] = u.z; v[3] = u.w;
}
CX_DEVICE void store4_bf16_sum(bf16_t* p, const float (&v)[4], float (&dc)[4]) {
    float r[4];
    unpack4_bf16(store4_bf16(p, v), r);
#pragma unroll
    for (int e = 0; e < 4; ++e) dc[e] += r[e];
}
template <int N>
CX_DEVICE void zero_acc(float (&a)[N][4]) {
#pragma unroll
    for (int i = 0; i < N; ++i)
#pragma unroll
        for (int e = 0; e < 4; ++e) a[i][e] = 0.f;
}
template <int NCH>
CX_DEVICE void fetch_row(const bf16_t* __restrict__ base, int row, int lane, uint2 (&raw)[NCH]) {
#pragma unroll
    for (int i = 0; i < NCH; ++i)
        raw[i] = *reinterpret_cast<const uint2*>(base + (size_t)row * (NCH * 256) + (i * 64 + lane) * 4);
}

CX_DEVICE float wave_mean(float v, int d) { return wave_sum(v) / (float)d; }

template <int NCH>
CX_DEVICE void row_stats(const float (&z)[NCH][4], int d, float eps, float& mean, float& rstd) {
    float s = 0.f;
#pragma unroll
    for (int i = 0; i < NCH; ++i)
#pragma unroll
        for (int e = 0; e < 4; ++e) s += z[i][e];
    mean = wave_mean(s, d);
    float v = 0.f;
#pragma unroll
    for (int i = 0; i < NCH; ++i)
#pragma unroll
        for (int e = 0; e < 4; ++e) {
            const float c = z[i][e] - mean;
            v += c * c;
        }
    rstd = rsqrtf(wave_mean(v, d) + eps);
}

CX_DEVICE float ln_affine(float z, float mean, float rstd, float g, float b) { return (z - mean) * rstd * g + b; }
CX_DEVICE float ln_bwd_accum(float zz, float g, float dy, float mean, float rstd, float& s1, float& s2, float& dg, float& db) {
    const float xh = (zz - mean) * rstd;
    const float wdy = g * dy;
    s1 += wdy * xh;
    s2 += wdy;
    dg += dy * xh;
    db += dy;
    return xh;
}
CX_DEVICE float ln_bwd_dz(float g, float dy, float xh, float s1, float s2, float rstd) { return (g * dy - s1 * xh - s2) * rstd; }

template <int NCH>
__global__ __launch_bounds__(256) void ln_fwd_kernel(const bf16_t* __restrict__ x0, const bf16_t* __restrict__ res,
                                                     const float* __restrict__ gamma,
                                                     const float* __restrict__ beta, bf16_t* __restrict__ out,
                                                     bf16_t* z_out, float* __restrict__ mean_o,
                                                     float* __restrict__ rstd_o, int rows, float eps) {
    constexpr int D = NCH * 256;
    const int lane = threadIdx.x & 63, wave = threadIdx.x >> 6;
    float g[NCH][4], b[NCH][4];
#pragma unroll
    for (int i = 0; i < NCH; ++i) {
        load4_f32(gamma + (i * 64 + lane) * 4, g[i]);
        load4_f32(beta + (i * 64 + lane) * 4, b[i]);
    }
    const int stride = gridDim.x * 4;
    int row = blockIdx.x * 4 + wave;
    uint2 nx[NCH], nr[NCH];
    if (row < rows) {
        fetch_row<NCH>(x0, row, lane, nx);
        if (res) fetch_row<NCH>(res, row, lane, nr);
    }
    for (; row < rows; row += stride) {
        float z[NCH][4];
#pragma unroll
        for (int i = 0; i < NCH; ++i) {
            unpack4_bf16(nx[i], z[i]);
            if (res) {
                float r[4];
                unpack4_bf16(nr[i], r);
#pragma unroll
                for (int e = 0; e < 4; ++e) z[i][e] += r[e];
            }
        }
        if (row + stride < rows) {
            fetch_row<NCH>(x0, row + stride, lane, nx);
            if (res) fetch_row<NCH>(res, row + stride, lane, nr);
        }
        float mean, rstd;
        row_stats<NCH>(z, D, eps, mean, rstd);
#pragma unroll
        for (int i = 0; i < NCH; ++i) {
            const size_t off = (size_t)row * D + (i * 64 + lane) * 4;
// ... 968 lines not shown
```

contrastors_amd/loss.py:

```python
from __future__ import annotations

import contextlib
import logging
from typing import Dict, List, Optional

import numpy as np
import torch
import torch.distributed as dist

from . import _C
from .distributed import gather_with_grad
from .policy import GradCachePolicy
from .rand_state import RandContext


def _scale_of(logit_scale) -> tuple:
    if isinstance(logit_scale, (int, float)):
        return float(logit_scale), None
    p = getattr(logit_scale, "logit_scale", None)
    if p is None:
        raise TypeError("logit_scale must be a LogitScale module or a number")
    const = getattr(logit_scale, "_const_scale", None)
    if const is not None and not p.requires_grad:
        return float(const), None
# ... 254 lines not shown
        kd_loss = similarity_kl_loss(student_q, student_d, teacher_q, teacher_d, temperature)
        infonce_loss = clip_loss(student_q, student_d, 50.0, gather_enabled=True)
        return {"loss": world * 1000 * kd_loss + infonce_loss, "kd_loss": kd_loss, "infonce_loss": infonce_loss}
    if loss_fn == "towers":
        scale = 1.0 / float(temperature)
        tq, td = teacher_q.detach(), teacher_d.detach()
        student = clip_loss(student_q, student_d, scale, gather_enabled=True)
        query = clip_loss(student_q, tq, scale, gather_enabled=True)
        document = clip_loss(student_d, td, scale, gather_enabled=True)
        teacher = clip_loss(student_q, td, scale, gather_enabled=True)
        return {"loss": (student + query + document + teacher) / 4, "loss_infonce_student": student,
                "loss_teacher_query": query, "loss_teacher_document": document, "loss_infonce_teacher": teacher}
    if loss_fn == "stella":
        raise NotImplementedError("distill_loss_fn 'stella': its triplet term differences every pair of pairwise scores "
                                  "(sc/trainers/distill.py:302-307, 406-410), O(N^4) memory in the reference's own form; "
                                  "served: mse, kd, towers")
    raise NotImplementedError(f"Loss function {loss_fn} not implemented")


def _split_inputs(inputs: Dict[str, torch.Tensor], chunk_size: int, tail_seqs: int = 0) -> List[Dict]:
    total = inputs["input_ids"].shape[0]
    lens = None
    mask = inputs.get("attention_mask")
    if "seqlens" in inputs:
        lens = inputs["seqlens"]
    elif mask is not None and mask.is_cuda:
        lens_t = mask.sum(-1)
        right_padded = (mask[:, 1:] <= mask[:, :-1]).all()
        host = torch.stack([lens_t.max(), right_padded.to(lens_t.dtype)]).cpu()
        lens = lens_t.cpu().numpy() if bool(host[1]) else None
    tail_seqs = max(0, min(int(tail_seqs), total))
    head = total - tail_seqs
    bounds = [(a, min(a + chunk_size, head)) for a in range(0, head, chunk_size)]
    tail = []
    e = total
    while e > head:
        tail.append((max(head, e - chunk_size), e))
        e -= chunk_size
    bounds += tail[::-1]
    chunks = []
    for a, b in bounds:
        c = {k: v[a:b] for k, v in inputs.items() if torch.is_tensor(v) and v.shape[0] == total}
        if lens is not None:
            c["seqlens"] = lens[a:b]
        chunks.append(c)
    return chunks


def _uses_rng(model) -> bool:
    trunk = getattr(model, "trunk", None)
    return bool(getattr(trunk, "uses_rng", False)) if trunk is not None else bool(getattr(model, "training", False))


def get_chunked_embeddings(model, chunks, rand_states=None, keep_tail: int = 0, kept: Optional[dict] = None):
    embs = []
    needed = rand_states is not None and _uses_rng(model)
    n = len(chunks)
    trainable = kept is not None and keep_tail > 0 and model.training and not getattr(model, "frozen_trunk", False)
    first_kept = n - keep_tail if trainable else n
    trunk = getattr(model, "trunk", None)
    for i, c in enumerate(chunks):
        if rand_states is not None:
            rand_states.append(RandContext(c, needed=needed))
        if i >= first_kept:
            suspended = (trunk.selective_checkpointing_suspended() if hasattr(trunk, "selective_checkpointing_suspended")
                         else contextlib.nullcontext())
            outstanding = getattr(trunk, "_outstanding", None)
            try:
                with torch.enable_grad(), suspended:
                    out = model(**c)["embedding"]
                kept[i] = out
                embs.append(out.detach())
                continue
            except torch.OutOfMemoryError:
                if outstanding is not None:
                    trunk._outstanding = outstanding
                first_kept = n
                if rand_states is not None:
                    rand_states[-1].restore()
                _log_once(("gradcache-tail-oom",), "GradCache: a kept chunk ran out of memory; the rest of the step re-forwards")
        with torch.no_grad():
            embs.append(model(**c)["embedding"])
    return torch.cat(embs, dim=0)


def accumulate_gradients(model, chunks, cache, rand_states=None, final: bool = False, skip=()):
    todo = [i for i in range(len(chunks)) if i not in skip]
    for i in todo:
        c, g = chunks[i], cache[i]
        state = rand_states[i] if rand_states is not None else RandContext(c, needed=False)
        if final and i == todo[-1] and hasattr(model, "arm_overlapped_reduce"):
            model.arm_overlapped_reduce()
        with state:
            out = model(**c)["embedding"]
        out.backward(g.to(out.dtype))


def cache_loss(query_embeddings, document_embeddings, logit_scale, bidirectional=False, *, use_fp8=False):
    q = query_embeddings.detach().requires_grad_()
    d = document_embeddings.detach().requires_grad_()
    loss = clip_loss(q, d, logit_scale, gather_enabled=True, bidirectional=bidirectional, use_fp8=use_fp8)
    loss.backward()
    return q.grad, d.grad, loss.detach()


_LOGGED: set = set()
LAST_SCHEDULE: dict = {}


def _log_once(key, msg: str):
    if key in _LOGGED:
        return
    _LOGGED.add(key)
    if not (dist.is_available() and dist.is_initialized()) or dist.get_rank() == 0:
        logging.getLogger("contrastors_amd").info(msg)


def effective_chunk(tower, inputs, chunk_size: int, policy: Optional[GradCachePolicy] = None) -> int:
    mode = (policy or GradCachePolicy()).with_env().chunk
    if mode == "exact" or chunk_size is None or chunk_size <= 0:
        return chunk_size
    if mode != "auto":
        return max(1, int(mode))
    cfg = getattr(getattr(tower, "trunk", None), "config", None)
    ids = inputs.get("input_ids") if isinstance(inputs, dict) else None
    if cfg is None or ids is None or ids.ndim != 2 or not ids.is_cuda:
        return chunk_size
    B, S = ids.shape
    bytes_per_token = _arena_bytes_per_token(tower)
    free, _ = torch.cuda.mem_get_info(ids.device)
    free += torch.cuda.memory_reserved(ids.device) - torch.cuda.memory_allocated(ids.device)
    free += sum(a.nbytes() for a in getattr(tower.trunk, "_arena_free", []))
    tokens = int(min(262144, max(S, free / 3 / bytes_per_token)))
    want = max(chunk_size, tokens // max(S, 1))
    want = max(chunk_size, want // chunk_size * chunk_size)
    return int(min(want, max(B, chunk_size)))


def _arena_bytes_per_token(tower) -> float:
    cfg = tower.trunk.config
    d, I, L = cfg.n_embd, cfg.n_inner, cfg.n_layer
    wfc1 = 2 * I if getattr(cfg, "gated", False) else I
    per_layer = 2 * (3 * d + 5 * d + I + I) + 4 * (cfg.n_head + 4)
    if getattr(cfg, "norm_mlp", False):
        per_layer += 2 * I + 4 * 2
    kept = 1 if getattr(tower.trunk, "gradient_checkpointing", False) else L
# ... 160 lines not shown
              f"({len(q_chunks)} + {len(d_chunks)} chunks; policy.chunk = {pol.chunk!r}); "
              f"{'pass 1 keeps its activations, no re-forward' if resident else 'two passes (re-forward)'} "
              f"(policy.resident = {pol.resident!r}); similarity GEMM {'fp8' if pol.use_fp8 else 'fp32'}")
    done = False
    fell_back = False
    LAST_SCHEDULE.clear()
    LAST_SCHEDULE.update(schedule="resident" if resident else ("partial" if (kq_seqs or kd_seqs) else "two-pass"),
                         chunk_q=cq, chunk_d=cd, chunks_q=len(q_chunks), chunks_d=len(d_chunks), kept_q_seqs=kq_seqs,
                         kept_d_seqs=kd_seqs, fell_back=False)
    if resident:
        q_out = d_out = None
        try:
            q_out = _resident_forward(tower1, q_chunks)
            d_out = _resident_forward(tower2, d_chunks)
        except torch.OutOfMemoryError:
            _release_resident(tower1, q_out)
            _release_resident(tower2, d_out)
            q_out = d_out = None
            if pol.resident is True:
                raise
            fell_back = True
            LAST_SCHEDULE.update(schedule="two-pass", fell_back=True)
            for tw in {id(tower1): tower1, id(tower2): tower2}.values():
                drop = getattr(getattr(tw, "trunk", None), "drop_idle_arenas", None)
                if drop is not None:
                    drop()
            torch.cuda.empty_cache()
            ids_ = t1_inputs.get("input_ids") if isinstance(t1_inputs, dict) else None
            if ids_ is not None and ids_.is_cuda:
                note_local_memory_shortfall(ids_.device, [tower1, tower2])
            _log_once(("gradcache-oom",), "GradCache: resident activations ran out of memory; falling back to the two-pass "
                                          "schedule (set train_args.gradcache_resident: false to skip the attempt)")
        else:
            try:
                q_cache, d_cache, loss = cache_loss(torch.cat([o.detach() for o in q_out]), torch.cat([o.detach() for o in d_out]),
                                                    logit_scale, bidirectional=bidirectional, use_fp8=pol.use_fp8)
            except torch.OutOfMemoryError:
                _release_resident(tower1, q_out)
                _release_resident(tower2, d_out)
                raise
            _resident_backward(tower1, q_out, q_cache.split(sizes_q), final=tower1 is not tower2 or not was_training2)
            _resident_backward(tower2, d_out, d_cache.split(sizes_d), final=True)
            del q_out, d_out
            done = True
    if not done:
        nq_keep = 0 if fell_back else (kq_seqs + cq - 1) // cq if kq_seqs else 0
        nd_keep = 0 if fell_back else (kd_seqs + cd - 1) // cd if kd_seqs else 0
        if nq_keep or nd_keep:
            _log_once(("gradcache-tail", len(q_chunks), len(d_chunks), kq_seqs, kd_seqs),
                      f"GradCache schedule: the last {kq_seqs} query and {kd_seqs} document sequences ({nq_keep} + {nd_keep} chunks of "
                      f"{len(q_chunks)} + {len(d_chunks)}) keep their activations (no re-forward for them)")
        q_rnd, d_rnd = [], []
        q_kept, d_kept = {}, {}
        try:
            q_embs = get_chunked_embeddings(tower1, q_chunks, q_rnd, keep_tail=nq_keep, kept=q_kept)
            d_embs = get_chunked_embeddings(tower2, d_chunks, d_rnd, keep_tail=nd_keep, kept=d_kept)
            q_cache, d_cache, loss = cache_loss(q_embs, d_embs, logit_scale, bidirectional=bidirectional, use_fp8=pol.use_fp8)
        except BaseException:
            _release_resident(tower1, list(q_kept.values()))
            _release_resident(tower2, list(d_kept.values()))
            raise
        q_grads, d_grads = q_cache.split(sizes_q), d_cache.split(sizes_d)
        done_q, done_d = set(q_kept), set(d_kept)
        re_q = len(done_q) < len(q_chunks)
        re_d = was_training2 and len(done_d) < len(d_chunks)
        shared = tower1 is tower2
        for i in sorted(done_q):
            o = q_kept.pop(i)
            last_of_tower1 = not re_q and not q_kept and (not shared or (not done_d and not re_d))
            if last_of_tower1 and hasattr(tower1, "arm_overlapped_reduce"):
                tower1.arm_overlapped_reduce()
            o.backward(q_grads[i].to(o.dtype))
        for i in sorted(done_d):
            o = d_kept.pop(i)
            last_of_tower2 = not re_d and not d_kept and not (shared and re_q)
            if last_of_tower2 and hasattr(tower2, "arm_overlapped_reduce"):
                tower2.arm_overlapped_reduce()
            o.backward(d_grads[i].to(o.dtype))
        if re_q:
            accumulate_gradients(tower1, q_chunks, q_grads, q_rnd, final=(not shared) or not re_d, skip=done_q)
        if re_d:
            accumulate_gradients(tower2, d_chunks, d_grads, d_rnd, final=True, skip=done_d)
    seen = set()
    for tw, active in ((tower1, was_training1), (tower2, was_training2)):
        if active and id(tw) not in seen and hasattr(tw, "sync_gradients"):
            seen.add(id(tw))
            tw.sync_gradients()
    return loss


def _release_resident(tower, outs):
    if not outs:
        return
    for o in outs:
        fn = getattr(o, "grad_fn", None)
        eng, arena = getattr(fn, "engine", None), getattr(fn, "arena", None)
        if eng is not None and arena is not None and hasattr(eng, "abandon_arena"):
            eng.abandon_arena(arena)
            fn.arena = None
```

contrastors_amd/nomic_bert.py:

```python
from __future__ import annotations

import contextlib
import ctypes as C
import logging
import math
import os
from dataclasses import dataclass
from typing import Dict, List, Optional, Tuple, Union

import numpy as np
import torch
import torch.distributed as dist

from . import _C
from .policy import _parse_keep


@dataclass
class NomicBertConfig:

    vocab_size: int = 30528
    n_positions: int = 2048
    n_embd: int = 768
    n_layer: int = 12
# ... 107 lines not shown
        t["qkv"] = torch.empty(n_slots, T_cap, 3 * d, **bf)
        t["ctx"] = torch.empty(n_slots, T_cap, d, **bf)
        t["lse"] = torch.empty(n_slots, T_cap * H, **f32)
        for n in ("z1", "h1", "z2", "h2"):
            t[n] = torch.empty(n_layer_slots if n == kept else n_slots, T_cap, d, **bf)
        for n in ("mean1", "rstd1", "mean2", "rstd2"):
            t[n] = torch.empty(n_slots, T_cap, **f32)
        t["yg"] = torch.empty(n_slots, T_cap, I, **bf)
        t["act"] = torch.empty(n_slots, T_cap, I, **bf)
        t["pool_norm"] = torch.empty(B_cap, **f32)
        patch_dim = int(getattr(cfg, "patch_dim", 0) or 0)
        if getattr(cfg, "prenorm", False):
            t["zf"] = torch.empty(T_cap, d, **bf)
            t["hf"] = torch.empty(T_cap, d, **bf)
            t["meanf"] = torch.empty(T_cap, **f32)
            t["rstdf"] = torch.empty(T_cap, **f32)
        if patch_dim:
            t["patch_in"] = torch.empty(T_cap, patch_dim, **bf)
            t["patch_proj"] = torch.empty(T_cap, d, **bf)
        if getattr(cfg, "prepre_layernom", False):
            t["zpre"] = torch.empty(T_cap, d, **bf)
        if getattr(cfg, "norm_mlp", False):
            t["sub_z"] = torch.empty(n_slots, T_cap, I, **bf)
            t["sub_mean"] = torch.empty(n_slots, T_cap, **f32)
            t["sub_rstd"] = torch.empty(n_slots, T_cap, **f32)
            if not with_backward:
                t["yg_wide"] = torch.empty(T_cap, 2 * I, **bf)
        ws_floats = max(8 * max(3 * d, wfc1, patch_dim) * d, 16 * d * d)
        if with_backward and wfc1 == I:
            ws_floats = max(ws_floats, ((T_cap + 127) // 128) * I)
        t["ws_f32"] = torch.empty(ws_floats, **f32)
        if with_backward:
            wide = max(3 * d, wfc1, patch_dim)
            for n in ("g_a", "g_b", "g_c"):
                t[n] = torch.empty(T_cap, d, **bf)
            t["g_wide"] = torch.empty(T_cap, wide, **bf)
            t["g_act"] = torch.empty(T_cap, I, **bf)
            if any(f % 256 for f in (d, 3 * d, I, wfc1) + ((patch_dim,) if patch_dim else ())):
                t["tr_a"] = torch.empty(wide, T_cap, **bf)
                t["tr_b"] = torch.empty(wide, T_cap, **bf)
            t["delta"] = torch.empty(T_cap * H, **f32)
            if getattr(cfg, "resid_pdrop", 0.0) > 0:
                t["g_d"] = torch.empty(T_cap, d, **bf)
        self.tensors = t
        self.desc = _C.CxChunkBuffers()
        self.desc.T_cap = T_cap
        for name, _ in _C.CxChunkBuffers._fields_[1:]:
            if name == "ws_floats":
                self.desc.ws_floats = t["ws_f32"].numel() if "ws_f32" in t else 0
            elif name == "checkpoint":
                self.desc.checkpoint = int(self.checkpoint)
            elif name == "ckpt_keep":
                self.desc.ckpt_keep = int(self.keep_layers)
            elif name in ("drop_active", "drop_seed", "drop_offset", "n_keep", "n_patch_all"):
                setattr(self.desc, name, 0)
            else:
                setattr(self.desc, name, t[name].data_ptr() if name in t else None)
        self.emb_out: Optional[torch.Tensor] = None

    def nbytes(self) -> int:
        return sum(x.numel() * x.element_size() for x in self.tensors.values())

    @staticmethod
    def slot_bytes_per_token(cfg) -> int:
        d, I, H = cfg.n_embd, cfg.n_inner, cfg.n_head
        extra = 2 * I + 4 * 2 if getattr(cfg, "norm_mlp", False) else 0
        return 2 * (3 * d + d + 3 * d + I + I) + 4 * (H + 4) + extra


_FULL_CACHE: Dict[tuple, tuple] = {}


@dataclass
class VarlenBatch:

    input_ids: torch.Tensor
    indices: torch.Tensor
    cu_seqlens: torch.Tensor
    B: int
    S: int
    T: int
    max_seqlen: int
    _sort: Optional[tuple] = None
    token_type_ids: Optional[torch.Tensor] = None

    def with_token_types(self, token_type_ids: Optional[torch.Tensor]) -> "VarlenBatch":
        if token_type_ids is not None:
            if token_type_ids.shape != self.input_ids.shape or token_type_ids.dtype != torch.int64 \
                    or token_type_ids.device != self.input_ids.device:
                raise ValueError("token_type_ids must be an int64 tensor of input_ids' shape on its device")
            token_type_ids = token_type_ids.contiguous()
        self.token_type_ids = token_type_ids
        return self

    def embedding_sort(self):
        if self._sort is None:
            import os

            if os.environ.get("CX_EMBED_ATOMICS"):
                self._sort = (None, None)
                return self._sort
            tok = self.input_ids.reshape(-1)[self.indices.long()].to(torch.int32)
            sorted_ids, perm = torch.sort(tok, stable=True)
            self._sort = (sorted_ids.contiguous(), perm.to(torch.int32).contiguous())
        return self._sort

    @staticmethod
    def from_lengths(input_ids: torch.Tensor, seqlens) -> "VarlenBatch":
        B, S = input_ids.shape
        lens = np.asarray(seqlens, dtype=np.int64).reshape(B)
        dev = input_ids.device
        full = bool((lens == S).all())
        if full:
            hit = _FULL_CACHE.get((B, S, str(dev)))
            if hit is not None:
                return VarlenBatch(input_ids, hit[0], hit[1], B, S, B * S, S)
        cu = np.zeros(B + 1, dtype=np.int32)
        np.cumsum(lens, out=cu[1:])
        T = int(cu[-1])
        if full:
# ... 15 lines not shown
        lens = mask.sum(-1, dtype=torch.int32)
        idx = torch.nonzero(mask.flatten(), as_tuple=False).flatten().to(torch.int32)
        cu = torch.zeros(B + 1, dtype=torch.int32, device=input_ids.device)
        cu[1:] = torch.cumsum(lens, 0)
        return VarlenBatch(input_ids, idx, cu, B, S, int(idx.numel()), int(lens.max().item()) if B else 0)


class NomicBertEngine(torch.nn.Module):

    def __init__(self, config: NomicBertConfig, device="cuda", pooling: str = "mean", normalize: bool = True,
                 seed: Optional[int] = None):
        super().__init__()
        self.config = config
        self.device_ = torch.device(device)
        if self.device_.type != "cuda":
            raise RuntimeError("NomicBertEngine needs an MI355X (cuda/hip device); there is no CPU path")
        self.lib = _C.lib()
        if pooling not in ("mean", "cls"):
            raise NotImplementedError(f"pooling={pooling}")
        self.pool_mode = 0 if pooling == "mean" else 1
        self.normalize_default = bool(normalize)
        decay, nodecay = self._param_specs()
        self._layout: Dict[str, Tuple[int, Tuple[int, ...]]] = {}
        off = 0
        for name, shape in decay:
            self._layout[name] = (off, shape)
            off += _round_up(int(np.prod(shape)), 64)
        self.n_decay = off
        for name, shape in nodecay:
            self._layout[name] = (off, shape)
            off += _round_up(int(np.prod(shape)), 64)
        self.n_total = off
        self._linear_names = [n for n, s in decay if self._is_linear(n)]
        self._lin_begin = self._layout[self._linear_names[0]][0]
        self._lin_end = self.n_decay

        dev = self.device_
        self.flat_param = torch.zeros(self.n_total, dtype=torch.float32, device=dev)
        self.flat_grad = torch.zeros(self.n_total, dtype=torch.float32, device=dev)
        self.flat_decay = torch.nn.Parameter(self.flat_param[: self.n_decay])
        self.flat_nodecay = torch.nn.Parameter(self.flat_param[self.n_decay:])
        self.flat_decay.grad = self.flat_grad[: self.n_decay]
        self.flat_nodecay.grad = self.flat_grad[self.n_decay:]
        n_lin = self._lin_end - self._lin_begin
        self.w16 = torch.zeros(n_lin, dtype=torch.bfloat16, device=dev)
        self.w16_t = torch.zeros(n_lin, dtype=torch.bfloat16, device=dev)

        self._init_weights(seed)
        self._build_rotary()
        self._build_desc()
        self._arena_nograd: Optional[_ChunkArena] = None
        self._arena_free: List[_ChunkArena] = []
        self._outstanding = 0
        self._overlap_armed = None
        self._ov_works = None
        self.gradient_checkpointing = False
        self.checkpoint_keep: Union[int, str] = 0
        self._keep_logged: set = set()
        self._keep_suspended = 0
        self._keep_plan: Dict[int, int] = {}
        self._keep_granted: Dict[int, int] = {}
        self._keep_granted_B: Dict[int, int] = {}
        self._arena_tick = 0
        self.sync_shadows()

    _LAYER_PREFIX = "encoder.layers.{l}."

    def _layer_specs(self, l: int):
        cfg = self.config
        d, I = cfg.n_embd, cfg.n_inner
        wfc1 = 2 * I if cfg.gated else I
        p = self._LAYER_PREFIX.format(l=l)
        decay = [(p + "attn.Wqkv.weight", (3 * d, d)), (p + "attn.out_proj.weight", (d, d)),
                 (p + "mlp.fc1_fused.weight", (wfc1, d)), (p + "mlp.fc2.weight", (d, I))]
        nodecay = []
        if cfg.qkv_proj_bias:
            nodecay += [(p + "attn.Wqkv.bias", (3 * d,)), (p + "attn.out_proj.bias", (d,))]
        if cfg.mlp_fc1_bias:
            nodecay.append((p + "mlp.fc1_fused.bias", (wfc1,)))
        if cfg.mlp_fc2_bias:
            nodecay.append((p + "mlp.fc2.bias", (d,)))
        nodecay += [(p + "norm1.weight", (d,)), (p + "norm1.bias", (d,)),
                    (p + "norm2.weight", (d,)), (p + "norm2.bias", (d,))]
        return decay, nodecay

    def _param_specs(self):
        cfg = self.config
        d = cfg.n_embd
        decay: List[Tuple[str, Tuple[int, ...]]] = [("embeddings.word_embeddings.weight", (cfg.vocab_size, d))]
        if cfg.rotary_emb_fraction == 0.0:
            decay.append(("embeddings.position_embeddings.weight", (cfg.max_position_embeddings, d)))
        decay.append(("embeddings.token_type_embeddings.weight", (cfg.type_vocab_size, d)))
        nodecay: List[Tuple[str, Tuple[int, ...]]] = [("emb_ln.weight", (d,)), ("emb_ln.bias", (d,))]
        for l in range(cfg.n_layer):
            dl, nl = self._layer_specs(l)
            decay += dl
            nodecay += nl
        return decay, nodecay

    def _is_linear(self, name: str) -> bool:
        return ".layers." in name or name.startswith("layers.")

    def p(self, name: str) -> torch.Tensor:
        off, shape = self._layout[name]
        return self.flat_param[off: off + int(np.prod(shape))].view(shape)

# ... 270 lines not shown
        free_now, _ = torch.cuda.mem_get_info(self.device_)
        free_now += torch.cuda.memory_reserved(self.device_) - torch.cuda.memory_allocated(self.device_) + arena.nbytes()
        budget = min(budget, self.CKPT_HBM_FRACTION * free_now - arena.nbytes() - _hbm_grant(self.device_, 0))
        keep = int(max(0, min(L, budget // max(per_keep, 1))))
        self._keep_plan[T_cap] = keep
        if keep == 0:
            return False
        _hbm_grant(self.device_, keep * per_keep)
        self._keep_granted[T_cap] = keep * per_keep
        self._keep_granted_B[T_cap] = int(getattr(arena, "B_cap", 0))
        return True

    @contextlib.contextmanager
    def selective_checkpointing_suspended(self):
        self._keep_suspended += 1
        try:
            yield
        finally:
            self._keep_suspended -= 1

    def _log_keep(self, T_cap: int, keep: int):
        key = (T_cap, keep)
        if key in self._keep_logged:
            return
        self._keep_logged.add(key)
        L = self.config.n_layer
        logging.getLogger("contrastors_amd").info(
            "selective checkpointing: %d-token arena keeps the activations of %d of %d blocks (%.1f GB), %d are recomputed "
            "in backward (checkpoint_keep_layers = %r)", T_cap, keep, L,
            keep * T_cap * _ChunkArena.slot_bytes_per_token(self.config) / 1e9, L - keep, self.checkpoint_keep)

    def _arm_dropout(self, arena: _ChunkArena):
        cfg = self.config
        active = self.training and any(getattr(cfg, k, 0.0) > 0 for k in ("resid_pdrop", "embd_pdrop", "attn_pdrop"))
        arena.desc.drop_active = int(active)
        if active:
            gen = torch.cuda.default_generators[self.device_.index if self.device_.index is not None else torch.cuda.current_device()]
            off = gen.get_offset()
            gen.set_offset(off + self.dropout_offset_stride(cfg.n_layer))
            arena.desc.drop_seed, arena.desc.drop_offset = gen.initial_seed() & (2**64 - 1), off

    @staticmethod
    def dropout_offset_stride(n_layer: int) -> int:
        return 4 * ((3 * n_layer + 1 + 3) // 4)

    @property
    def uses_rng(self) -> bool:
        cfg = self.config
        return self.training and any(getattr(cfg, k, 0.0) > 0 for k in ("resid_pdrop", "embd_pdrop", "attn_pdrop"))

    def release_arena(self, arena: _ChunkArena, used: bool = True):
        arena.emb_out = None
        arena.desc.layer_events = None
        if used and getattr(arena, "probation", False) and self._plan_keep(arena):
            return
        self._arena_free.append(arena)

    def abandon_arena(self, arena: _ChunkArena):
        self._outstanding = max(0, self._outstanding - 1)
        self.release_arena(arena, used=False)

    def grad_ranges(self):
        L = self.config.n_layer
        per_layer, covered = [], []
        for l in range(L):
            pre = self._LAYER_PREFIX.format(l=l)
            runs = []
            for lo, hi in ((0, self.n_decay), (self.n_decay, self.n_total)):
                offs = [(off, off + _round_up(int(np.prod(shape)), 64)) for n, (off, shape) in self._layout.items()
                        if n.startswith(pre) and lo <= off < hi]
                if offs:
                    a, b = min(o[0] for o in offs), max(o[1] for o in offs)
                    assert sum(o[1] - o[0] for o in offs) == b - a, "a block's parameters are contiguous per group"
                    runs.append((a, b))
            per_layer.append(runs)
            covered += runs
        covered.sort()
        tail, pos = [], 0
        for a, b in covered + [(self.n_total, self.n_total)]:
            if a > pos:
                tail.append((pos, a))
            pos = max(pos, b)
        return per_layer, tail

    def arm_overlapped_reduce(self, when_last_outstanding: bool = False):
        if not (dist.is_available() and dist.is_initialized() and dist.get_world_size() > 1):
            return
        self._overlap_armed = "last" if when_last_outstanding else "next"

    def _overlap_fires(self) -> bool:
        armed = getattr(self, "_overlap_armed", None)
        if armed == "next" or (armed == "last" and self._outstanding == 1):
            self._overlap_armed = None
            return True
        return False

    def _overlap_events(self):
        L = self.config.n_layer
        if getattr(self, "_ov_events", None) is None:
            self._ov_events = [torch.cuda.Event() for _ in range(L + 1)]
            for e in self._ov_events:
                e.record(torch.cuda.current_stream(self.device_))
            self._ov_handles = (C.c_void_p * (L + 1))(*[e.cuda_event for e in self._ov_events])
            self._ov_stream = torch.cuda.Stream(device=self.device_)
            self._ov_ranges = self.grad_ranges()
        return self._ov_events

    def _launch_overlapped_reduce(self):
        ev = self._ov_events
        per_layer, tail = self._ov_ranges
        works = []
        with torch.cuda.stream(self._ov_stream):
            for l in range(self.config.n_layer - 1, -1, -1):
                self._ov_stream.wait_event(ev[l])
                for a, b in per_layer[l]:
                    works.append(dist.all_reduce(self.flat_grad[a:b], op=dist.ReduceOp.SUM, async_op=True))
            self._ov_stream.wait_event(ev[self.config.n_layer])
            for a, b in tail:
                works.append(dist.all_reduce(self.flat_grad[a:b], op=dist.ReduceOp.SUM, async_op=True))
        self._ov_works = works

    def finish_overlapped_reduce(self) -> bool:
        works = getattr(self, "_ov_works", None)
        if not works:
            return False
        for w in works:
            w.wait()
        torch.cuda.current_stream(self.device_).wait_stream(self._ov_stream)
        self._ov_works = None
        return True

    def gradient_checkpointing_enable(self, enabled: bool = True, keep_layers: Union[int, str, None] = None):
        self.gradient_checkpointing = bool(enabled)
        if keep_layers is not None:
            self.checkpoint_keep = parse_checkpoint_keep(keep_layers, "checkpoint_keep_layers")
        self._arena_free = []

    def forward_chunk(self, vb: VarlenBatch, save_for_backward: bool, normalize: Optional[bool] = None,
                      out: Optional[torch.Tensor] = None) -> Tuple[torch.Tensor, Optional[_ChunkArena]]:
        d = self.config.n_embd
        if self.config.rotary_emb_fraction > 0 and self.config.rotary_scaling_factor:
            self._update_rotary(vb.max_seqlen)
        elif vb.S > (self.config.n_positions if self.rot_cos is not None else self.config.max_position_embeddings):
            raise ValueError("sequence longer than the position table")
        if out is None:
            out = torch.empty(vb.B, d, dtype=torch.float32, device=self.device_)
        arena = self._get_arena(vb.T, vb.B, save_for_backward)
        self._arm_dropout(arena)
        self._desc.normalize = int(self.normalize_default if normalize is None else normalize)
        if vb.token_type_ids is None:
            rc = self.lib.cx_encoder_forward(C.byref(self._desc), C.byref(arena.desc), vb.input_ids.data_ptr(),
                                             vb.indices.data_ptr(), vb.cu_seqlens.data_ptr(), vb.B, vb.S, vb.T,
                                             vb.max_seqlen, int(save_for_backward), out.data_ptr(), _C.cur_stream())
            _C.check(rc, "cx_encoder_forward")
        else:
            self._check_token_types()
            rc = self.lib.cx_encoder_forward_typed(C.byref(self._desc), C.byref(arena.desc), vb.input_ids.data_ptr(),
                                                   vb.token_type_ids.data_ptr(), vb.indices.data_ptr(),
                                                   vb.cu_seqlens.data_ptr(), vb.B, vb.S, vb.T, vb.max_seqlen,
                                                   int(save_for_backward), out.data_ptr(), _C.cur_stream())
            _C.check(rc, "cx_encoder_forward_typed")
        if save_for_backward:
            arena.emb_out = out
            arena.normalize = self._desc.normalize
            self._outstanding += 1
            return out, arena
        return out, None

    def _check_token_types(self):
        if self.config.type_vocab_size != 2:
            raise NotImplementedError(f"token_type_ids need type_vocab_size == 2 (the config has {self.config.type_vocab_size})")

    def drop_idle_arenas(self):
        for a in self._arena_free:
            self._keep_plan.pop(a.T_cap, None)
        self._arena_free = []
        self._arena_nograd = None
        torch.cuda.empty_cache()

    def backward_chunk(self, vb: VarlenBatch, arena: _ChunkArena, demb: torch.Tensor):
        assert arena.emb_out is not None, "backward_chunk needs a forward with save_for_backward=True"
        demb = demb.to(torch.float32).contiguous()
        self._desc.normalize = arena.normalize
        sids, perm = vb.embedding_sort()
        fires = self._begin_backward(arena)
        if vb.token_type_ids is None:
            rc = self.lib.cx_encoder_backward(C.byref(self._desc), C.byref(arena.desc), vb.input_ids.data_ptr(),
                                              vb.indices.data_ptr(), vb.cu_seqlens.data_ptr(), vb.B, vb.S, vb.T,
                                              vb.max_seqlen, demb.data_ptr(), arena.emb_out.data_ptr(), _C.ptr(sids),
                                              _C.ptr(perm), _C.cur_stream())
            _C.check(rc, "cx_encoder_backward")
        else:
            rc = self.lib.cx_encoder_backward_typed(C.byref(self._desc), C.byref(arena.desc), vb.input_ids.data_ptr(),
                                                    vb.token_type_ids.data_ptr(), vb.indices.data_ptr(),
                                                    vb.cu_seqlens.data_ptr(), vb.B, vb.S, vb.T, vb.max_seqlen,
                                                    demb.data_ptr(), arena.emb_out.data_ptr(), _C.ptr(sids), _C.ptr(perm),
                                                    _C.cur_stream())
            _C.check(rc, "cx_encoder_backward_typed")
        self._end_backward(arena, fires)

    def _begin_backward(self, arena: _ChunkArena) -> bool:
        fires = self._overlap_fires()
        if fires:
            self._overlap_events()
            arena.desc.layer_events = C.cast(self._ov_handles, C.POINTER(C.c_void_p))
        return fires

    def _end_backward(self, arena: _ChunkArena, fires: bool):
        self._outstanding = max(0, self._outstanding - 1)
        if fires:
            self._launch_overlapped_reduce()
        self.release_arena(arena)

    def _rotary_or_bounds(self, vb: VarlenBatch):
        if self.config.rotary_emb_fraction > 0 and self.config.rotary_scaling_factor:
            self._update_rotary(vb.max_seqlen)
        elif vb.S > (self.config.n_positions if self.rot_cos is not None else self.config.max_position_embeddings):
            raise ValueError("sequence longer than the position table")

    def forward_hidden_chunk(self, vb: VarlenBatch, save_for_backward: bool):
# ... 65 lines not shown
```

contrastors_amd/policy.py:

```python
from __future__ import annotations

import os
from dataclasses import dataclass
from typing import Union


@dataclass
class GradCachePolicy:
    chunk: Union[str, int] = "auto"
    resident: Union[str, bool] = "auto"
    use_fp8: bool = False

    @classmethod
    def from_train_args(cls, ta) -> "GradCachePolicy":
        return cls(chunk=_parse_chunk(getattr(ta, "gradcache_chunk", "auto"), "train_args.gradcache_chunk"),
                   resident=_parse_resident(getattr(ta, "gradcache_resident", "auto"), "train_args.gradcache_resident"),
                   use_fp8=bool(getattr(ta, "use_fp8", False)))

    def with_env(self) -> "GradCachePolicy":
        c, r = os.environ.get("CX_GRADCACHE_CHUNK"), os.environ.get("CX_GRADCACHE_RESIDENT")
        return GradCachePolicy(chunk=self.chunk if c in (None, "") else _parse_chunk(c, "CX_GRADCACHE_CHUNK"),
                               resident=self.resident if r in (None, "") else _parse_resident(r, "CX_GRADCACHE_RESIDENT"),
                               use_fp8=self.use_fp8)


def _parse_chunk(v, where: str):
    if v is None or v == "":
        return "auto"
    if isinstance(v, str) and v.lower() in ("auto", "exact"):
        return v.lower()
    try:
        n = int(v)
    except (TypeError, ValueError):
        raise ValueError(f"{where} must be 'auto', 'exact' or a positive integer, got {v!r}") from None
    if n <= 0:
        raise ValueError(f"{where} must be 'auto', 'exact' or a positive integer, got {v!r}")
    return n


def _parse_resident(v, where: str):
    if v is None or v == "":
        return "auto"
    if isinstance(v, bool):
        return v
    t = str(v).lower()
    if t == "auto":
        return "auto"
    if t in ("1", "true", "yes", "on"):
        return True
    if t in ("0", "false", "no", "off"):
        return False
    raise ValueError(f"{where} must be 'auto', true / 1 or false / 0, got {v!r}")


def _parse_keep(v, where: str):
    if v is None or v == "":
        return "auto"
    if isinstance(v, str) and v.strip().lower() == "auto":
        return "auto"
    if isinstance(v, bool):
        raise ValueError(f"{where} must be 'auto' or a non-negative integer, got {v!r}")
    try:
        n = int(v)
    except (TypeError, ValueError):
        raise ValueError(f"{where} must be 'auto' or a non-negative integer, got {v!r}") from None
    if n < 0:
        raise ValueError(f"{where} must be 'auto' or a non-negative integer, got {v!r}")
    return n
```

include/contrastors_hip.h:

```cpp
#ifndef CONTRASTORS_HIP_H
#define CONTRASTORS_HIP_H

#include <stdint.h>

#ifdef __cplusplus
extern "C" {
#endif

#define CX_OK 0
#define CX_ERR_SHAPE (-1)
#define CX_ERR_ALIGN (-2)
#define CX_ERR_ARG (-3)
#define CX_ERR_LAUNCH (-4)

int cx_abi_version(void);
const char* cx_build_info(void);
const char* cx_error_string(int code);

int cx_gemm_bf16_nt(const uint16_t* X, const uint16_t* W, void* Out, const float* bias, int M, int N, int K, int ldx,
                    int ldw, int ldo, int out_mode, int split_k, float alpha, void* stream);
int cx_gemm_bf16_nt_accum(const uint16_t* X, const uint16_t* W, float* Out, float* ws, long ws_floats, int M, int N,
                          int K, int ldx, int ldw, void* stream);
int cx_gemm_bf16_tn_accum(const uint16_t* dY, const uint16_t* A, float* G, float* ws, long ws_floats, int T, int O, int I,
                          int ld_dy, int ld_a, void* stream);
// ... 34 lines not shown
                                 float p, unsigned long long seed, unsigned long long offset, unsigned int site,
                                 void* stream);
int cx_dropout_add_layernorm_bwd(const uint16_t* dout_a, const uint16_t* dout_b, const uint16_t* z, const float* gamma,
                                 const float* mean, const float* rstd, uint16_t* dz, uint16_t* dx0, float* dgamma,
                                 float* dbeta, float* ws, long ws_floats, int rows, int d, float p,
                                 unsigned long long seed, unsigned long long offset, unsigned int site, void* stream);
int cx_dropout_add_layernorm_bwd_colsum(const uint16_t* dout_a, const uint16_t* dout_b, const uint16_t* z, const float* gamma,
                                        const float* mean, const float* rstd, uint16_t* dz, uint16_t* dx0, float* dgamma, float* dbeta,
                                        float* dx0_colsum, float* ws, long ws_floats, int rows, int d, float p, unsigned long long seed,
                                        unsigned long long offset, unsigned int site, void* stream);
int cx_dropout_scale(uint16_t* x, long n, float p, unsigned long long seed, unsigned long long offset, unsigned int site,
                     void* stream);

int cx_layernorm_fwd_mixed(const void* x0, const void* residual, const float* gamma, const float* beta, void* out,
                           void* z_out, float* mean, float* rstd, int rows, int d, float eps, int flags, void* stream);
int cx_layernorm_bwd_mixed(const void* dout, const void* z, const float* gamma, const float* mean, const float* rstd,
                           const void* dz_extra, void* dx0, void* dres, float* dgamma, float* dbeta, int rows, int d,
                           int flags, void* stream);

int cx_embed_ln_fwd(const int64_t* input_ids, const int32_t* indices, const float* word, const float* type0,
                    const float* pos_emb, const float* gamma, const float* beta, uint16_t* out, float* mean,
                    float* rstd, int T, int S, int d, float eps, void* stream);
int cx_embed_ln_bwd(const uint16_t* dout_a, const uint16_t* dout_b, const int64_t* input_ids,
                    const int32_t* indices, const float* word, const float* type0, const float* pos_emb,
                    const float* gamma, const float* mean, const float* rstd, float* dword, float* dtype0,
                    float* dpos, float* dgamma, float* dbeta, int T, int S, int d, int padding_idx, void* stream);

int cx_embed_ln_bwd_sorted(const uint16_t* dout_a, const uint16_t* dout_b, const int64_t* input_ids,
                           const int32_t* indices, const float* word, const float* type0, const float* pos_emb,
                           const float* gamma, const float* mean, const float* rstd, float* dword, float* dtype0,
                           float* dpos, float* dgamma, float* dbeta, int T, int S, int d, int padding_idx, int vocab,
                           const int32_t* sorted_ids, const int32_t* perm, float* dz_scratch, void* stream);

int cx_embed_ln_fwd_typed(const int64_t* input_ids, const int64_t* token_type_ids, const int32_t* indices, const float* word,
                          const float* type, int type_vocab_size, const float* pos_emb, const float* gamma, const float* beta,
                          uint16_t* out, float* mean, float* rstd, int T, int S, int d, float eps, void* stream);
int cx_embed_ln_bwd_typed(const uint16_t* dout_a, const uint16_t* dout_b, const int64_t* input_ids,
                          const int64_t* token_type_ids, const int32_t* indices, const float* word, const float* type,
                          int type_vocab_size, const float* pos_emb, const float* gamma, const float* mean, const float* rstd,
                          float* dword, float* dtype, float* dpos, float* dgamma, float* dbeta, float* ws, long ws_floats, int T,
                          int S, int d, int padding_idx, void* stream);
int cx_embed_ln_bwd_sorted_typed(const uint16_t* dout_a, const uint16_t* dout_b, const int64_t* input_ids,
                                 const int64_t* token_type_ids, const int32_t* indices, const float* word, const float* type,
                                 int type_vocab_size, const float* pos_emb, const float* gamma, const float* mean,
                                 const float* rstd, float* dword, float* dtype, float* dpos, float* dgamma, float* dbeta,
                                 float* ws, long ws_floats, int T, int S, int d, int padding_idx, int vocab,
                                 const int32_t* sorted_ids, const int32_t* perm, float* dz_scratch, void* stream);

int cx_swiglu_fwd(const uint16_t* yg, uint16_t* act, int T, int I, int layout, void* stream);
int cx_swiglu_bwd(const uint16_t* dact, const uint16_t* yg, uint16_t* dyg, int T, int I, int layout, void* stream);
int cx_gemm_bf16_nt_residual(const uint16_t* X, const uint16_t* W, uint16_t* Out, const float* bias,
                             const uint16_t* Residual, int M, int N, int K, int ldx, int ldw, int ldo, int ldr,
                             void* stream);
int cx_gemm_bf16_nt_splitk(const uint16_t* X, const uint16_t* W, uint16_t* Out, const float* bias, const uint16_t* Residual,
                           float* ws, long ws_floats, int M, int N, int K, int ldx, int ldw, int ldo, int ldr, void* stream);
int cx_gemm_bf16_swiglu(const uint16_t* X, const uint16_t* W, uint16_t* YG, uint16_t* Act, int M, int I, int K, int ldx,
                        int ldw, int ld_yg, int ld_act, void* stream);
int cx_gemm_bf16_bias_gelu(const uint16_t* X, const uint16_t* W, const float* bias, uint16_t* Pre, uint16_t* Act, int M,
                           int N, int K, int ldx, int ldw, int ld_pre, int ld_act, void* stream);
int cx_gemm_bf16_bias_act(const uint16_t* X, const uint16_t* W, const float* bias, uint16_t* Pre, uint16_t* Act, int M,
                          int N, int K, int ldx, int ldw, int ld_pre, int ld_act, int act, void* stream);
int cx_gemm_bf16_act_bwd(const uint16_t* dY, const uint16_t* W, const uint16_t* Pre, uint16_t* dPre, float* dbias, float* ws,
                         long ws_floats, int M, int N, int K, int ldx, int ldw, int ld_pre, int ld_dpre, int act, void* stream);
int cx_gemm_bf16_swiglu_bwd(const uint16_t* dY, const uint16_t* W, const uint16_t* YG, uint16_t* dYG, int M, int I, int K,
                            int ldx, int ldw, int ld_yg, void* stream);
int cx_gemm_bf16_swiglu_gate(const uint16_t* X, const uint16_t* W, uint16_t* G, uint16_t* Act, int M, int I, int K, int ldx,
                             int ldw, int ld_g, int ld_act, void* stream);
int cx_gemm_bf16_swiglu_bwd_gate(const uint16_t* dY, const uint16_t* W, const uint16_t* Act, const uint16_t* G, uint16_t* dYG,
                                 int M, int I, int K, int ldx, int ldw, int ld_ag, int ld_dyg, void* stream);
int cx_swiglu_bwd_gate(const uint16_t* dact, const uint16_t* act, const uint16_t* gate, uint16_t* dyg, int T, int I,
                       void* stream);
int cx_bias_gelu_fwd(const uint16_t* pre, const float* bias, uint16_t* act, int T, int I, void* stream);
int cx_bias_gelu_bwd(const uint16_t* dact, const uint16_t* pre, const float* bias, uint16_t* dpre, int T, int I,
                     void* stream);
int cx_bias_gelu_bwd_colsum(const uint16_t* dact, const uint16_t* pre, const float* bias, uint16_t* dpre, float* dbias, int T,
                            int I, void* stream);
int cx_bias_act_fwd(const uint16_t* pre, const float* bias, uint16_t* act_out, int T, int I, int act, void* stream);
int cx_bias_act_bwd_colsum(const uint16_t* dact, const uint16_t* pre, const float* bias, uint16_t* dpre, float* dbias, int T,
                           int I, int act, void* stream);
int cx_bias_grad(const uint16_t* dY, float* dbias, int T, int N, int ld, void* stream);

int cx_attn_varlen_fwd(const uint16_t* qkv, const int32_t* cu_seqlens, const float* rot_cos, const float* rot_sin,
                       uint16_t* out, float* lse, int B, int H, int T, int max_seqlen, float softmax_scale,
                       void* stream);
int cx_attn_varlen_bwd(const uint16_t* dout, const uint16_t* qkv, const uint16_t* out, const float* lse,
                       const int32_t* cu_seqlens, const float* rot_cos, const float* rot_sin, float* delta,
                       uint16_t* dqkv, int B, int H, int T, int max_seqlen, float softmax_scale, void* stream);

int cx_attn_varlen_bwd_prerotated(const uint16_t* dout, const uint16_t* qkv_rotated, const uint16_t* out, const float* lse,
                                  const int32_t* cu_seqlens, const float* rot_cos, const float* rot_sin, float* delta,
                                  uint16_t* dqkv, int B, int H, int T, int max_seqlen, float softmax_scale, void* stream);

int cx_attn_varlen_dropout_fwd(const uint16_t* qkv, const int32_t* cu_seqlens, const float* rot_cos, const float* rot_sin,
                               uint16_t* out, float* lse, int B, int H, int T, int max_seqlen, float softmax_scale,
                               float p_drop, unsigned long long seed, unsigned long long offset, unsigned int site,
                               void* stream);
int cx_attn_varlen_dropout_bwd(const uint16_t* dout, const uint16_t* qkv, const uint16_t* out, const float* lse,
                               const int32_t* cu_seqlens, const float* rot_cos, const float* rot_sin, float* delta,
                               uint16_t* dqkv, int B, int H, int T, int max_seqlen, float softmax_scale, float p_drop,
                               unsigned long long seed, unsigned long long offset, unsigned int site, void* stream);

int cx_attn_varlen_kvpacked_fwd(const uint16_t* q, const uint16_t* kv, const int32_t* cu_seqlens_q,
                                const int32_t* cu_seqlens_k, uint16_t* out, float* lse, int B, int H, int Tq,
                                int max_seqlen_q, int max_seqlen_k, float softmax_scale, void* stream);
int cx_attn_varlen_kvpacked_bwd(const uint16_t* dout, const uint16_t* q, const uint16_t* kv, const uint16_t* out,
                                const float* lse, const int32_t* cu_seqlens_q, const int32_t* cu_seqlens_k, float* delta,
// ... 125 lines not shown
    int pool_mode, normalize;
    int prenorm;
    const float* lnf_g; const float* lnf_b;
    float* glnf_g; float* glnf_b;
    const uint16_t* Wpatch;
    const float* bpatch;
    const float* cls_token;
    const float* vit_pos;
    float* gWpatch; float* gbpatch; float* gcls_token; float* gvit_pos;
    int patch_dim;
    float resid_pdrop, embd_pdrop;
    float attn_pdrop;
    int mlp_act;
    const float* lnpre_g; const float* lnpre_b;
    float* glnpre_g; float* glnpre_b;
} CxEncoderDesc;

typedef struct CxChunkBuffers {
    long T_cap;
    uint16_t* h0;
    float* emb_mean; float* emb_rstd;
    uint16_t* qkv;
    uint16_t* ctx;
    float* lse;
    uint16_t* z1;
    uint16_t* h1;
    float* mean1; float* rstd1;
    uint16_t* yg;
    uint16_t* act;
    uint16_t* z2;
    uint16_t* h2;
    float* mean2; float* rstd2;
    float* pool_norm;
    uint16_t* g_a; uint16_t* g_b; uint16_t* g_c;
    uint16_t* g_wide;
    uint16_t* g_act;
    uint16_t* tr_a; uint16_t* tr_b;
    float* delta;
    float* ws_f32;
    long ws_floats;
    uint16_t* zf; uint16_t* hf; float* meanf; float* rstdf;
    uint16_t* patch_in; uint16_t* patch_proj;
    int checkpoint;
    int drop_active;
    unsigned long long drop_seed, drop_offset;
    uint16_t* g_d;
    void* const* layer_events;
    uint16_t* zpre;
    int ckpt_keep;
    const int32_t* patch_keep;
    const int32_t* patch_inv;
    int n_keep;
    int n_patch_all;
} CxChunkBuffers;

int cx_encoder_forward(const CxEncoderDesc* enc, const CxChunkBuffers* buf, const int64_t* input_ids,
                       const int32_t* indices, const int32_t* cu_seqlens, int Bc, int S, int T, int max_seqlen,
                       int save_for_backward, float* emb_out, void* stream);
int cx_encoder_backward(const CxEncoderDesc* enc, const CxChunkBuffers* buf, const int64_t* input_ids,
                        const int32_t* indices, const int32_t* cu_seqlens, int Bc, int S, int T, int max_seqlen,
                        const float* demb, const float* emb_out, const int32_t* sort_ids, const int32_t* sort_perm,
                        void* stream);

int cx_encoder_forward_typed(const CxEncoderDesc* enc, const CxChunkBuffers* buf, const int64_t* input_ids,
                             const int64_t* token_type_ids, const int32_t* indices, const int32_t* cu_seqlens, int Bc, int S,
                             int T, int max_seqlen, int save_for_backward, float* emb_out, void* stream);
int cx_encoder_backward_typed(const CxEncoderDesc* enc, const CxChunkBuffers* buf, const int64_t* input_ids,
                              const int64_t* token_type_ids, const int32_t* indices, const int32_t* cu_seqlens, int Bc, int S,
                              int T, int max_seqlen, const float* demb, const float* emb_out, const int32_t* sort_ids,
                              const int32_t* sort_perm, void* stream);

int cx_encoder_forward_hidden(const CxEncoderDesc* enc, const CxChunkBuffers* buf, const int64_t* input_ids,
                              const int32_t* indices, const int32_t* cu_seqlens, int Bc, int S, int T, int max_seqlen,
                              int save_for_backward, uint16_t* hidden_out, void* stream);
int cx_encoder_backward_hidden(const CxEncoderDesc* enc, const CxChunkBuffers* buf, const int64_t* input_ids,
                               const int32_t* indices, const int32_t* cu_seqlens, int Bc, int S, int T, int max_seqlen,
                               const uint16_t* dhidden, const int32_t* sort_ids, const int32_t* sort_perm, void* stream);

int cx_vit_patchify(const void* pixels, int pixels_bf16, uint16_t* patches, int B, int C, int H, int W, int patch,
                    void* stream);
int cx_vit_assemble_fwd(const uint16_t* proj, const float* cls_token, const float* pos_embed, uint16_t* out, int B,
                        int P, int d, void* stream);
int cx_vit_assemble_bwd(const uint16_t* dz, uint16_t* dproj, float* gcls, float* gpos, int B, int P, int d,
                        void* stream);
int cx_vit_patchify_gather(const void* pixels, int pixels_bf16, uint16_t* patches, int B, int C, int H, int W, int patch,
                           const int32_t* keep, int n_keep, void* stream);
int cx_vit_assemble_fwd_gather(const uint16_t* proj, const float* cls_token, const float* pos_embed, uint16_t* out, int B,
                               int P, int d, const int32_t* keep, void* stream);
int cx_vit_assemble_bwd_gather(const uint16_t* dz, uint16_t* dproj, float* gcls, float* gpos, int B, int P, int d,
                               const int32_t* inv, int P_all, void* stream);
int cx_vit_forward(const CxEncoderDesc* enc, const CxChunkBuffers* buf, const void* pixels, int pixels_bf16,
                   const int32_t* cu_seqlens, int Bc, int C, int H, int W, int patch, int save_for_backward,
                   float* emb_out, void* stream);
int cx_vit_backward(const CxEncoderDesc* enc, const CxChunkBuffers* buf, const int32_t* cu_seqlens, int Bc,
                    int n_patch, const float* demb, const float* emb_out, void* stream);
int cx_vit_forward_hidden(const CxEncoderDesc* enc, const CxChunkBuffers* buf, const void* pixels, int pixels_bf16,
                          const int32_t* cu_seqlens, int Bc, int Cc, int H, int W, int patch, int save_for_backward,
                          uint16_t* hidden_out, void* stream);
int cx_vit_backward_hidden(const CxEncoderDesc* enc, const CxChunkBuffers* buf, const int32_t* cu_seqlens, int Bc, int n_patch,
                           const uint16_t* dhidden, void* stream);

int cx_rope2d_qkv_inplace(uint16_t* qkv, const int32_t* cu_seqlens, const float* rope_cos, const float* rope_sin, int n_rope,
                          int B, int n_head, int T, int n_prefix, int sign, void* stream);
int cx_swiglu_subln_fwd(const uint16_t* yg, const float* gamma, const float* beta, uint16_t* gate, uint16_t* act, uint16_t* z,
                        float* mean, float* rstd, int T, int I, float eps, void* stream);
int cx_swiglu_subln_bwd(const uint16_t* dz, const uint16_t* act, const uint16_t* gate, const float* mean, const float* rstd,
// ... 58 lines not shown
```

Before: 4370.

## Reuse LayerNorm statistics from no-grad pass to fuse LN into residual GEMM epilogue

During GradCache, the no-grad forward now records the per-layer LayerNorm mean and rstd into a persistent store. The grad-enabled re-forward reads them back and applies LN directly inside the output-projection GEMM epilogue (residual add plus affine normalize). This removes the separate layernorm kernels and their row reductions from the re-forward, for post-norm models without checkpointing or residual dropout. It costs extra memory for the stats buffers, relies on the two passes seeing identical inputs (checked by chunk identity), and may change numerics slightly because the stats come from the earlier pass.

```diff
diff --git a/contrastors_amd/_C.py b/contrastors_amd/_C.py
--- a/contrastors_amd/_C.py
+++ b/contrastors_amd/_C.py
@@ -58,7 +58,8 @@
             "h2", "mean2", "rstd2", "pool_norm", "g_a", "g_b", "g_c", "g_wide", "g_act", "tr_a", "tr_b", "delta",
             "ws_f32",
         )
-    ] + [("ws_floats", i64)] + [(n, vp) for n in ("zf", "hf", "meanf", "rstdf", "patch_in", "patch_proj")] + [("checkpoint", i32), ("drop_active", i32), ("drop_seed", C.c_ulonglong), ("drop_offset", C.c_ulonglong), ("g_d", vp), ("layer_events", C.POINTER(vp)), ("zpre", vp), ("ckpt_keep", i32), ("patch_keep", vp), ("patch_inv", vp), ("n_keep", i32), ("n_patch_all", i32)]
+    ] + [("ws_floats", i64)] + [(n, vp) for n in ("zf", "hf", "meanf", "rstdf", "patch_in", "patch_proj")] + [("checkpoint", i32), ("drop_active", i32), ("drop_seed", C.c_ulonglong), ("drop_offset", C.c_ulonglong), ("g_d", vp), ("layer_events", C.POINTER(vp)), ("zpre", vp), ("ckpt_keep", i32), ("patch_keep", vp), ("patch_inv", vp), ("n_keep", i32), ("n_patch_all", i32),
+                                  ("ln_stats_in", vp), ("ln_stats_out", vp), ("ln_stats_stride", i64)]
 
 
 
@@ -108,6 +109,8 @@
     "cx_swiglu_bwd": (i32, [vp, vp, vp, i32, i32, i32, vp]),
     "cx_gemm_bf16_swiglu": (i32, [vp, vp, vp, vp, i32, i32, i32, i32, i32, i32, i32, vp]),
     "cx_gemm_bf16_nt_residual": (i32, [vp, vp, vp, vp, vp, i32, i32, i32, i32, i32, i32, i32, vp]),
+    "cx_gemm_bf16_nt_residual_ln": (i32, [vp] * 10 + [i32] * 8 + [vp]),
+    "cx_gemm_bf16_nt_residual_ln_min_tiles": (i32, []),
     "cx_gemm_bf16_swiglu_bwd": (i32, [vp, vp, vp, vp, i32, i32, i32, i32, i32, i32, vp]),
     "cx_gemm_bf16_nt_splitk": (i32, [vp, vp, vp, vp, vp, vp, i64, i32, i32, i32, i32, i32, i32, i32, vp]),
     "cx_gemm_bf16_swiglu_gate": (i32, [vp, vp, vp, vp, i32, i32, i32, i32, i32, i32, i32, vp]),
diff --git a/contrastors_amd/config.py b/contrastors_amd/config.py
--- a/contrastors_amd/config.py
+++ b/contrastors_amd/config.py
@@ -44,6 +44,7 @@
     use_fp8: Optional[bool] = False
     gradcache_chunk: Union[int, str, None] = "auto"
     gradcache_resident: Union[bool, str, None] = "auto"
+    gradcache_ln_stats: bool = True
     exchange: Optional[str] = "auto"
     exchange_timeout_s: float = 120.0
     overlap_grad_reduce: bool = True
diff --git a/contrastors_amd/csrc/engine.hip b/contrastors_amd/csrc/engine.hip
--- a/contrastors_amd/csrc/engine.hip
+++ b/contrastors_amd/csrc/engine.hip
@@ -24,6 +24,10 @@
     int d, I, wfc1;
     int mode;
     int first_kept;
+    float* stats = nullptr;
+    long sstride = 0;
+    bool stats_in = false;
+    float* stat(int s, int which) const { return stats + ((size_t)s * 4 + which) * sstride; }
     bool kept(int s) const { return mode == 1 || (mode == 2 && s >= first_kept); }
     int sl(int s) const { return mode == 1 ? s : (mode == 2 && s >= first_kept) ? 1 + s - first_kept : 0; }
     int sl_in(int s) const { return mode == 0 ? 0 : s; }
@@ -32,14 +36,14 @@
     float* lse(int s) const { return b->lse + (size_t)sl(s) * T_cap * e->n_head; }
     uint16_t* z1(int s) const { return b->z1 + (size_t)(e->prenorm ? sl_in(s) : sl(s)) * T_cap * d; }
     uint16_t* h1(int s) const { return b->h1 + (size_t)sl(s) * T_cap * d; }
-    float* mean1(int s) const { return b->mean1 + (size_t)sl(s) * T_cap; }
-    float* rstd1(int s) const { return b->rstd1 + (size_t)sl(s) * T_cap; }
+    float* mean1(int s) const { return stats ? stat(s, 0) : b->mean1 + (size_t)sl(s) * T_cap; }
+    float* rstd1(int s) const { return stats ? stat(s, 1) : b->rstd1 + (size_t)sl(s) * T_cap; }
     uint16_t* yg(int s) const { return b->yg + (size_t)sl(s) * T_cap * I; }
     uint16_t* act(int s) const { return b->act + (size_t)sl(s) * T_cap * I; }
     uint16_t* z2(int s) const { return b->z2 + (size_t)sl(s) * T_cap * d; }
     uint16_t* h2(int s) const { return b->h2 + (size_t)(e->prenorm ? sl(s) : sl_in(s)) * T_cap * d; }
-    float* mean2(int s) const { return b->mean2 + (size_t)sl(s) * T_cap; }
-    float* rstd2(int s) const { return b->rstd2 + (size_t)sl(s) * T_cap; }
+    float* mean2(int s) const { return stats ? stat(s, 2) : b->mean2 + (size_t)sl(s) * T_cap; }
+    float* rstd2(int s) const { return stats ? stat(s, 3) : b->rstd2 + (size_t)sl(s) * T_cap; }
     uint16_t* ez(const CxVitExt* x, int s) const { return x->z + (size_t)sl(s) * T_cap * I; }
     float* ezmean(const CxVitExt* x, int s) const { return x->zmean + (size_t)sl(s) * T_cap; }
     float* ezrstd(const CxVitExt* x, int s) const { return x->zrstd + (size_t)sl(s) * T_cap; }
@@ -62,8 +66,17 @@
 Slots make_slots(const CxEncoderDesc* enc, const CxChunkBuffers* buf, int save) {
     const int L = enc->n_layer;
     int keep = buf->ckpt_keep < 0 ? 0 : buf->ckpt_keep > L ? L : buf->ckpt_keep;
-    return Slots{buf, enc, buf->T_cap, enc->d, enc->d_inner, enc->gated ? 2 * enc->d_inner : enc->d_inner,
-                 save ? (buf->checkpoint ? 2 : 1) : 0, L - keep};
+    Slots s{buf, enc, buf->T_cap, enc->d, enc->d_inner, enc->gated ? 2 * enc->d_inner : enc->d_inner,
+            save ? (buf->checkpoint ? 2 : 1) : 0, L - keep};
+    const bool carry = !enc->prenorm && !buf->checkpoint && !(buf->drop_active && enc->resid_pdrop > 0.f);
+    if (carry && save && buf->ln_stats_in) {
+        s.stats = const_cast<float*>(buf->ln_stats_in);
+        s.stats_in = true;
+    } else if (carry && !save && buf->ln_stats_out) {
+        s.stats = buf->ln_stats_out;
+    }
+    s.sstride = buf->ln_stats_stride;
+    return s;
 }
 
 int check_desc(const CxEncoderDesc* e, const CxChunkBuffers* b, int T) {
@@ -72,6 +85,7 @@
     if (e->d != e->n_head * 64) return CX_ERR_SHAPE;
     if ((e->d % 64) != 0 || (e->d_inner % 64) != 0) return CX_ERR_SHAPE;
     if (b->T_cap < round_up(T, 64)) return CX_ERR_SHAPE;
+    if ((b->ln_stats_in || b->ln_stats_out) && b->ln_stats_stride < T) return CX_ERR_SHAPE;
     return CX_OK;
 }
 
@@ -96,9 +110,23 @@
     return cx_gemm_bf16_nt_accum(b->tr_a, b->tr_b, gW, b->ws_f32, b->ws_floats, out_f, in_f, Tp, Tp, Tp, stream);
 }
 
+struct LnFromStats {
+    const float* mean; const float* rstd; const float* gamma; const float* beta;
+    uint16_t* h;
+    bool keep_z;
+    bool done = false;
+};
 int proj_residual(const uint16_t* x, const uint16_t* W, const float* bias, const uint16_t* residual, uint16_t* out, int T,
-                  int N, int K, bool* folded, void* stream, const CxChunkBuffers* buf = nullptr) {
+                  int N, int K, bool* folded, void* stream, const CxChunkBuffers* buf = nullptr, LnFromStats* ln = nullptr) {
     *folded = false;
+    if (ln && residual) {
+        const int rc = cx_gemm_bf16_nt_residual_ln(x, W, ln->keep_z ? out : nullptr, ln->h, bias, residual, ln->mean, ln->rstd, ln->gamma,
+                                                   ln->beta, T, N, K, K, K, N, N, N, stream);
+        if (rc != CX_ERR_SHAPE) {
+            *folded = ln->done = rc == CX_OK;
+            return rc;
+        }
+    }
     if (buf && buf->ws_f32 && (long)((T + 255) / 256) * ((N + 255) / 256) <= 64 && K >= 1536) {
         const int rc = cx_gemm_bf16_nt_splitk(x, W, out, bias, residual, buf->ws_f32, buf->ws_floats, T, N, K, K, K, N, N, stream);
         if (rc != CX_ERR_SHAPE) {
@@ -148,11 +176,12 @@
         return cx_bias_act_fwd(s.yg(l), w.bfc1, s.act(l), T, I, enc->mlp_act, stream);
     }
     int mlp(const CxLayerWeights& w, const uint16_t* x, int l, uint16_t* out, const uint16_t* residual, bool keep,
-            bool* folded) const {
+            bool* folded, LnFromStats* ln = nullptr) const {
         CX_TRY(mlp_up(w, x, l, keep));
-        return proj_residual(ext_subln(ext) ? s.ez(ext, l) : s.act(l), w.Wfc2, w.bfc2, residual, out, T, enc->d, enc->d_inner, folded, stream, buf);
-    }
-    int attn(const CxLayerWeights& w, const uint16_t* x, int l, uint16_t* out, const uint16_t* residual, bool* folded) const {
+        return proj_residual(ext_subln(ext) ? s.ez(ext, l) : s.act(l), w.Wfc2, w.bfc2, residual, out, T, enc->d, enc->d_inner, folded, stream, buf, ln);
+    }
+    int attn(const CxLayerWeights& w, const uint16_t* x, int l, uint16_t* out, const uint16_t* residual, bool* folded,
+             LnFromStats* ln = nullptr) const {
         const int d = enc->d;
         CX_TRY(cx_gemm_bf16_nt(x, w.Wqkv, s.qkv(l), w.bqkv, T, 3 * d, d, d, d, 3 * d, 0, 1, 1.f, stream));
         if (ext_rope(ext))
@@ -171,7 +200,7 @@
             CX_TRY(cx_attn_varlen_fwd(s.qkv(l), cu_seqlens, enc->rot_cos, enc->rot_sin, s.ctx(l), s.lse(l), Bc, enc->n_head, T,
                                       max_seqlen, enc->softmax_scale, stream));
         }
-        return proj_residual(s.ctx(l), w.Wout, w.bout, residual, out, T, d, d, folded, stream);
+        return proj_residual(s.ctx(l), w.Wout, w.bout, residual, out, T, d, d, folded, stream, nullptr, ln);
     }
     int post_block(int l, const uint16_t* h_in, bool keep) const {
         const CxLayerWeights& w = enc->layers[l];
@@ -187,10 +216,14 @@
                                                 s.rstd2(l), T, d, enc->ln_eps, p, buf->drop_seed, buf->drop_offset, 2 * l + 1,
                                                 stream);
         }
-        CX_TRY(attn(w, h_in, l, s.z1(l), h_in, &f1));
-        CX_TRY(cx_layernorm_fwd(s.z1(l), f1 ? nullptr : h_in, w.ln1_g, w.ln1_b, s.h1(l), (keep && !f1) ? s.z1(l) : nullptr,
-                                s.mean1(l), s.rstd1(l), T, d, enc->ln_eps, stream));
-        CX_TRY(mlp(w, s.h1(l), l, s.z2(l), s.h1(l), keep, &f2));
+        const bool from_stats = s.stats_in && !ext;
+        LnFromStats ln1{s.mean1(l), s.rstd1(l), w.ln1_g, w.ln1_b, s.h1(l), keep}, ln2{s.mean2(l), s.rstd2(l), w.ln2_g, w.ln2_b, s.h2(l), keep};
+        CX_TRY(attn(w, h_in, l, s.z1(l), h_in, &f1, from_stats ? &ln1 : nullptr));
+        if (!ln1.done)
+            CX_TRY(cx_layernorm_fwd(s.z1(l), f1 ? nullptr : h_in, w.ln1_g, w.ln1_b, s.h1(l), (keep && !f1) ? s.z1(l) : nullptr,
+                                    s.mean1(l), s.rstd1(l), T, d, enc->ln_eps, stream));
+        CX_TRY(mlp(w, s.h1(l), l, s.z2(l), s.h1(l), keep, &f2, from_stats ? &ln2 : nullptr));
+        if (ln2.done) return CX_OK;
         return cx_layernorm_fwd(s.z2(l), f2 ? nullptr : s.h1(l), w.ln2_g, w.ln2_b, s.h2(l), (keep && !f2) ? s.z2(l) : nullptr,
                                 s.mean2(l), s.rstd2(l), T, d, enc->ln_eps, stream);
     }
diff --git a/contrastors_amd/csrc/gemm_api.hip b/contrastors_amd/csrc/gemm_api.hip
--- a/contrastors_amd/csrc/gemm_api.hip
+++ b/contrastors_amd/csrc/gemm_api.hip
@@ -189,6 +189,23 @@
     return cx_launch_gemm_v6(p, GEMM_EPI_NONE, (hipStream_t)stream) == hipSuccess ? CX_OK : CX_ERR_LAUNCH;
 }
 
+int cx_gemm_bf16_nt_residual_ln(const uint16_t* X, const uint16_t* W, uint16_t* Z, uint16_t* H, const float* bias,
+                                const uint16_t* Residual, const float* Mean, const float* Rstd, const float* Gamma,
+                                const float* Beta, int M, int N, int K, int ldx, int ldw, int ldz, int ldr, int ldh, void* stream) {
+    if (M <= 0 || N <= 0) return CX_OK;
+    if (!Residual || !H || !Mean || !Rstd || !Gamma || !Beta) return CX_ERR_ARG;
+    if (bias || K <= 0 || (K % 64) != 0 || (Z && (ldz % 8) != 0) || (ldr % 8) != 0 || (ldh % 8) != 0) return CX_ERR_SHAPE;
+    if ((ldx % 8) != 0 || (ldw % 8) != 0 || (((uintptr_t)Gamma | (uintptr_t)Beta) & 15) != 0) return CX_ERR_ALIGN;
+    GemmParams p = base_params(X, W, Z, nullptr, M, N, K, ldx, ldw, ldz);
+    p.Out2 = const_cast<uint16_t*>(Residual); p.ldo2 = ldr;
+    p.OutH = H; p.ldh = ldh;
+    p.ln_mean = Mean; p.ln_rstd = Rstd; p.ln_gamma = Gamma; p.ln_beta = Beta;
+    if (!cx_gemm_v6_resid_ln_covers(p)) return CX_ERR_SHAPE;
+    ProfScope prof(2.0 * (double)M * (double)N * (double)K, (hipStream_t)stream);
+    return cx_launch_gemm_v6(p, GEMM_EPI_RESID_LN, (hipStream_t)stream) == hipSuccess ? CX_OK : CX_ERR_LAUNCH;
+}
+int cx_gemm_bf16_nt_residual_ln_min_tiles(void) { return cx_gemm_v6_resid_ln_min_tiles(); }
+
 int cx_gemm_bf16_bias_gelu(const uint16_t* X, const uint16_t* W, const float* bias, uint16_t* Pre, uint16_t* Act, int M, int N,
                            int K, int ldx, int ldw, int ld_pre, int ld_act, void* stream) {
     return cx_gemm_bf16_bias_act(X, W, bias, Pre, Act, M, N, K, ldx, ldw, ld_pre, ld_act, 0, stream);
diff --git a/contrastors_amd/csrc/gemm_bf16.hip b/contrastors_amd/csrc/gemm_bf16.hip
--- a/contrastors_amd/csrc/gemm_bf16.hip
+++ b/contrastors_amd/csrc/gemm_bf16.hip
@@ -821,6 +821,26 @@
     return e == hipSuccess ? CX_OK : CX_ERR_LAUNCH;
 }
 
+int cx_gemm_bf16_nt_residual_ln(const uint16_t* X, const uint16_t* W, uint16_t* Z, uint16_t* H, const float* bias,
+                                const uint16_t* Residual, const float* Mean, const float* Rstd, const float* Gamma,
+                                const float* Beta, int M, int N, int K, int ldx, int ldw, int ldz, int ldr, int ldh, void* stream) {
+    if (M <= 0 || N <= 0) return CX_OK;
+    if (!Residual || !H || !Mean || !Rstd || !Gamma || !Beta) return CX_ERR_ARG;
+    if (bias || K <= 0 || (K % 64) != 0 || (Z && (ldz % 8) != 0) || (ldr % 8) != 0 || (ldh % 8) != 0) return CX_ERR_SHAPE;
+    if ((ldx % 8) != 0 || (ldw % 8) != 0 || (((uintptr_t)Gamma | (uintptr_t)Beta) & 15) != 0) return CX_ERR_ALIGN;
+    if (cx_gemm_get_variant() != 6) return CX_ERR_SHAPE;
+    GemmParams p = {};
+    p.X = X; p.W = W; p.Out = Z;
+    p.M = M; p.N = N; p.K = K; p.ldx = ldx; p.ldw = ldw; p.ldo = ldz;
+    p.split_k = 1; p.alpha = 1.f;
+    p.Out2 = const_cast<uint16_t*>(Residual); p.ldo2 = ldr;
+    p.OutH = H; p.ldh = ldh;
+    p.ln_mean = Mean; p.ln_rstd = Rstd; p.ln_gamma = Gamma; p.ln_beta = Beta;
+    if (!cx_gemm_v6_resid_ln_covers(p)) return CX_ERR_SHAPE;
+    return cx_launch_gemm_v6(p, GEMM_EPI_RESID_LN, (hipStream_t)stream) == hipSuccess ? CX_OK : CX_ERR_LAUNCH;
+}
+int cx_gemm_bf16_nt_residual_ln_min_tiles(void) { return cx_gemm_v6_resid_ln_min_tiles(); }
+
 int cx_gemm_bf16_bias_gelu(const uint16_t* X, const uint16_t* W, const float* bias, uint16_t* Pre, uint16_t* Act, int M,
                            int N, int K, int ldx, int ldw, int ld_pre, int ld_act, void* stream) {
     return cx_gemm_bf16_bias_act(X, W, bias, Pre, Act, M, N, K, ldx, ldw, ld_pre, ld_act, 0, stream);
diff --git a/contrastors_amd/csrc/gemm_bf16_v6.hip b/contrastors_amd/csrc/gemm_bf16_v6.hip
--- a/contrastors_amd/csrc/gemm_bf16_v6.hip
+++ b/contrastors_amd/csrc/gemm_bf16_v6.hip
@@ -1,6 +1,7 @@
 #include "cx_common.h"
 #include "../../include/contrastors_hip.h"
 #include "gemm_params.h"
+#include "ln_affine.h"
 #include <type_traits>
 
 namespace {
@@ -308,7 +309,7 @@
             auto pcol = [&](int q) { return (q & 1) * 16 + 4 * g4; };
             auto qoff = [](int q, int rowb) { return (q >> 1) * 16 * rowb + (q & 1) * 32; };
             if constexpr ((DBG & 16) != 0) {
-            } else if constexpr (EPI == GEMM_EPI_NONE || EPI == GEMM_EPI_ACT_BWD || EPI == GEMM_EPI_QACT_BWD) {
+            } else if constexpr (EPI == GEMM_EPI_NONE || EPI == GEMM_EPI_ACT_BWD || EPI == GEMM_EPI_QACT_BWD || EPI == GEMM_EPI_RESID_LN) {
                 constexpr bool ACTB = EPI == GEMM_EPI_ACT_BWD || EPI == GEMM_EPI_QACT_BWD;
                 float cs0 = 0.f, cs1 = 0.f, cs2 = 0.f, cs3 = 0.f, cs4 = 0.f, cs5 = 0.f, cs6 = 0.f, cs7 = 0.f;
                 constexpr int act_kind = EPI == GEMM_EPI_QACT_BWD ? CX_ACT_QUICK_GELU : CX_ACT_GELU;
@@ -342,13 +343,35 @@
                 };
                 const bool add_bias = p.bias != nullptr;
                 const bf16_t* resid = reinterpret_cast<const bf16_t*>(p.Out2);
-                auto fast_tile = [&](auto with_resid) {
-                    constexpr bool RES = decltype(with_resid)::value;
+                auto fast_tile = [&](auto mode) {
+                    constexpr bool RES = decltype(mode)::value >= 1, LN = decltype(mode)::value == 2;
                     const int rrow = lane >> 4, rch = lane & 15;
                     bf16_t* outp = reinterpret_cast<bf16_t*>(p.Out) + (size_t)(m0 + rrow) * p.ldo + n0 + rch * 8;
                     const bf16_t* resp = RES ? resid + (size_t)(m0 + rrow) * p.ldo2 + n0 + rch * 8 : nullptr;
                     const char* rd = my + rrow * ROWB + rch * 16;
                     char* wr = my + prow(0) * ROWB + pcol(0) * 2;
+                    float4 lg0 = {}, lg1 = {}, lb0 = {}, lb1 = {};
+                    float mu_lo = 0.f, mu_hi = 0.f, rs_lo = 0.f, rs_hi = 0.f;
+                    bf16_t* outh = nullptr;
+                    if constexpr (LN) {
+                        outh = reinterpret_cast<bf16_t*>(p.OutH) + (size_t)(m0 + rrow) * p.ldh + n0 + rch * 8;
+                        lg0 = *reinterpret_cast<const float4*>(p.ln_gamma + n0 + rch * 8);
+                        lg1 = *reinterpret_cast<const float4*>(p.ln_gamma + n0 + rch * 8 + 4);
+                        lb0 = *reinterpret_cast<const float4*>(p.ln_beta + n0 + rch * 8);
+                        lb1 = *reinterpret_cast<const float4*>(p.ln_beta + n0 + rch * 8 + 4);
+                        mu_lo = p.ln_mean[m0 + lane]; mu_hi = p.ln_mean[m0 + 64 + lane];
+                        rs_lo = p.ln_rstd[m0 + lane]; rs_hi = p.ln_rstd[m0 + 64 + lane];
+                        __builtin_amdgcn_sched_barrier(0);
+                    }
+                    auto ln_row = [&](uint4& v, int b, int i) {
+                        const int src = ((b & 1) * 32 + 4 * i + rrow) * 4;
+                        const float mu = __int_as_float(__builtin_amdgcn_ds_bpermute(src, __float_as_int(b < 2 ? mu_lo : mu_hi)));
+                        const float rs = __int_as_float(__builtin_amdgcn_ds_bpermute(src, __float_as_int(b < 2 ? rs_lo : rs_hi)));
+                        v.x = pack_bf16x2(ln_affine(bf16lo_to_f32(v.x), mu, rs, lg0.x, lb0.x), ln_affine(bf16hi_to_f32(v.x), mu, rs, lg0.y, lb0.y));
+                        v.y = pack_bf16x2(ln_affine(bf16lo_to_f32(v.y), mu, rs, lg0.z, lb0.z), ln_affine(bf16hi_to_f32(v.y), mu, rs, lg0.w, lb0.w));
+                        v.z = pack_bf16x2(ln_affine(bf16lo_to_f32(v.z), mu, rs, lg1.x, lb1.x), ln_affine(bf16hi_to_f32(v.z), mu, rs, lg1.y, lb1.y));
+                        v.w = pack_bf16x2(ln_affine(bf16lo_to_f32(v.w), mu, rs, lg1.z, lb1.z), ln_affine(bf16hi_to_f32(v.w), mu, rs, lg1.w, lb1.w));
+                    };
                     uint2 pk[16];
                     auto pack_pass = [&](int b) {
 #pragma unroll
@@ -411,14 +434,24 @@
                             asm volatile("" ::"v"(o));
                             return;
                         }
-                        gst(o, v0);
-                        gst(o + (size_t)4 * p.ldo, v1);
-                        gst(o + (size_t)8 * p.ldo, v2);
-                        gst(o + (size_t)12 * p.ldo, v3);
-                        gst(o + (size_t)16 * p.ldo, v4);
-                        gst(o + (size_t)20 * p.ldo, v5);
-                        gst(o + (size_t)24 * p.ldo, v6);
-                        gst(o + (size_t)28 * p.ldo, v7);
+                        auto store_rows = [&](bf16_t* o_, int ld_) {
+                            gst(o_, v0);
+                            gst(o_ + (size_t)4 * ld_, v1);
+                            gst(o_ + (size_t)8 * ld_, v2);
+                            gst(o_ + (size_t)12 * ld_, v3);
+                            gst(o_ + (size_t)16 * ld_, v4);
+                            gst(o_ + (size_t)20 * ld_, v5);
+                            gst(o_ + (size_t)24 * ld_, v6);
+                            gst(o_ + (size_t)28 * ld_, v7);
+                        };
+                        if constexpr (LN) {
+                            if (p.Out) store_rows(o, p.ldo);
+                            ln_row(v0, b, 0); ln_row(v1, b, 1); ln_row(v2, b, 2); ln_row(v3, b, 3);
+                            ln_row(v4, b, 4); ln_row(v5, b, 5); ln_row(v6, b, 6); ln_row(v7, b, 7);
+                            store_rows(outh + (size_t)(b * 32) * p.ldh, p.ldh);
+                        } else {
+                            store_rows(o, p.ldo);
+                        }
                     };
                     if constexpr (RES) { CX_RES_ROWS(0) }
                     pack_pass(0);
@@ -550,7 +583,9 @@
                         }
                     }
                 };
-                if constexpr (ACTB) {
+                if constexpr (EPI == GEMM_EPI_RESID_LN) {
+                    fast_tile(std::integral_constant<int, 2>{});
+                } else if constexpr (ACTB) {
                     if (fast) {
                         fast_tile_actb();
                     } else {
@@ -559,9 +594,9 @@
                     flush_colsum();
                 } else if (fast) {
                     if (resid) {
-                        fast_tile(std::true_type{});
+                        fast_tile(std::integral_constant<int, 1>{});
                     } else {
-                        fast_tile(std::false_type{});
+                        fast_tile(std::integral_constant<int, 0>{});
                     }
                 } else if (p.alpha == 1.f && !add_bias) {
                     store_tile(std::true_type{});
@@ -1310,13 +1345,14 @@
 #else
 constexpr int g_v7_mode = -1;
 #endif
+constexpr long V7_MAX_TILES256 = 400;
 bool v7_takes(const GemmParams& p, int epi) {
     const int mode = g_v7_mode >= 0 ? (g_v7_mode ? 2 : 0) : CX_V7_POLICY;
     if (mode == 0 || !cx_gemm_v7_covers(p, epi)) return false;
     if (mode == 2) return true;
     if (epi == GEMM_EPI_SWIGLU_G) return false;
     const long tiles256 = (long)((p.M + BM6 - 1) / BM6) * ((p.N + BN6 - 1) / BN6);
-    return tiles256 <= 400;
+    return tiles256 <= V7_MAX_TILES256;
 }
 
 #ifndef CX_PRODUCT
@@ -1381,7 +1417,15 @@
     return hipGetLastError();
 }
 
+bool cx_gemm_v6_resid_ln_covers(const GemmParams& p) {
+    if ((p.M % BM6) != 0 || (p.N % BN6) != 0 || (p.K % BK6) != 0 || p.N / BN6 > 256) return false;
+    if (p.alpha != 1.f || p.bias || !p.Out2 || !p.OutH) return false;
+    return !v7_takes(p, GEMM_EPI_NONE);
+}
+int cx_gemm_v6_resid_ln_min_tiles(void) { return (int)V7_MAX_TILES256 + 1; }
+
 hipError_t cx_launch_gemm_v6(GemmParams p, int epi, hipStream_t stream) {
+    if (epi == GEMM_EPI_RESID_LN && !cx_gemm_v6_resid_ln_covers(p)) return hipErrorInvalidValue;
     if (v7_takes(p, epi)) return cx_launch_gemm_v7(p, epi, g_v6_force_gn, stream);
     p.tiles_m = (p.M + BM6 - 1) / BM6;
     p.tiles_n = (p.N + BN6 - 1) / BN6;
@@ -1420,6 +1464,7 @@
            : epi == GEMM_EPI_GELU ? launch6<GEMM_EPI_GELU>(p, stream)
            : epi == GEMM_EPI_QGELU ? launch6<GEMM_EPI_QGELU>(p, stream)
            : epi == GEMM_EPI_SWIGLU_BWD ? launch6<GEMM_EPI_SWIGLU_BWD>(p, stream)
+           : epi == GEMM_EPI_RESID_LN ? launch6<GEMM_EPI_RESID_LN>(p, stream)
            : epi == GEMM_EPI_ACT_BWD ? (p.act == CX_ACT_QUICK_GELU ? launch6<GEMM_EPI_QACT_BWD>(p, stream) : launch6<GEMM_EPI_ACT_BWD>(p, stream))
                                   : launch6<GEMM_EPI_NONE>(p, stream);
 }
diff --git a/contrastors_amd/csrc/gemm_params.h b/contrastors_amd/csrc/gemm_params.h
--- a/contrastors_amd/csrc/gemm_params.h
+++ b/contrastors_amd/csrc/gemm_params.h
@@ -8,6 +8,7 @@
        GEMM_EPI_SWIGLU_G = 5,
        GEMM_EPI_SWIGLU_BWD_AG = 6,
        GEMM_EPI_QACT_BWD = 8,
+       GEMM_EPI_RESID_LN = 9,
        GEMM_EPI_ACT_BWD = 7 };
 
 struct GemmParams {
@@ -27,10 +28,18 @@
     float* colsum_part;
     int sup_m, sup_n;
     long long* trace;
+    void* OutH;
+    int ldh;
+    const float* ln_mean;
+    const float* ln_rstd;
+    const float* ln_gamma;
+    const float* ln_beta;
 };
 
 hipError_t cx_launch_gemm_v5(GemmParams p, int form, int out_mode, int epi, hipStream_t stream);
 hipError_t cx_launch_gemm_v6(GemmParams p, int epi, hipStream_t stream);
+bool cx_gemm_v6_resid_ln_covers(const GemmParams& p);
+int cx_gemm_v6_resid_ln_min_tiles(void);
 void cx_gemm_v6_force_groups(int gn);
 void cx_gemm_v6_set_trace(long long* buf);
 void cx_gemm_v6_set_ablate(int mask);
diff --git a/contrastors_amd/csrc/layernorm.hip b/contrastors_amd/csrc/layernorm.hip
--- a/contrastors_amd/csrc/layernorm.hip
+++ b/contrastors_amd/csrc/layernorm.hip
@@ -1,5 +1,6 @@
 #include "cx_common.h"
 #include "ln_workspace.h"
+#include "ln_affine.h"
 #include "../../include/contrastors_hip.h"
 
 namespace {
@@ -61,7 +62,6 @@
     rstd = rsqrtf(wave_mean(v, d) + eps);
 }
 
-CX_DEVICE float ln_affine(float z, float mean, float rstd, float g, float b) { return (z - mean) * rstd * g + b; }
 CX_DEVICE float ln_bwd_accum(float zz, float g, float dy, float mean, float rstd, float& s1, float& s2, float& dg, float& db) {
     const float xh = (zz - mean) * rstd;
     const float wdy = g * dy;
diff --git a/contrastors_amd/csrc/ln_affine.h b/contrastors_amd/csrc/ln_affine.h
--- /dev/null
+++ b/contrastors_amd/csrc/ln_affine.h
@@ -0,0 +1,4 @@
+#pragma once
+#include "cx_common.h"
+
+CX_DEVICE float ln_affine(float z, float mean, float rstd, float g, float b) { return (z - mean) * rstd * g + b; }
diff --git a/contrastors_amd/loss.py b/contrastors_amd/loss.py
--- a/contrastors_amd/loss.py
+++ b/contrastors_amd/loss.py
@@ -330,7 +330,27 @@
     return bool(getattr(trunk, "uses_rng", False)) if trunk is not None else bool(getattr(model, "training", False))
 
 
-def get_chunked_embeddings(model, chunks, rand_states=None, keep_tail: int = 0, kept: Optional[dict] = None):
+def _ln_stats_side(model, side: str, policy: Optional[GradCachePolicy] = None):
+    trunk = getattr(model, "trunk", None)
+    if policy is not None and not policy.reforward_ln_stats:
+        return None
+    if trunk is None or not hasattr(trunk, "ln_stats_scope") or not model.training or getattr(model, "frozen_trunk", False):
+        return None
+    return None if _uses_rng(model) else (trunk, side)
+
+
+def _chunk_id(c) -> tuple:
+    return tuple((k, v.data_ptr(), tuple(v.shape), v._version) for k, v in sorted(c.items()) if isinstance(v, torch.Tensor))
+
+
+def _ln_stats_ctx(ln_stats, i: int, mode: str, c):
+    if ln_stats is None:
+        return contextlib.nullcontext()
+    trunk, side = ln_stats
+    return trunk.ln_stats_scope((side, i), mode, _chunk_id(c))
+
+
+def get_chunked_embeddings(model, chunks, rand_states=None, keep_tail: int = 0, kept: Optional[dict] = None, ln_stats=None):
     embs = []
     needed = rand_states is not None and _uses_rng(model)
     n = len(chunks)
@@ -345,7 +365,7 @@
                          else contextlib.nullcontext())
             outstanding = getattr(trunk, "_outstanding", None)
             try:
-                with torch.enable_grad(), suspended:
+                with torch.enable_grad(), suspended, _ln_stats_ctx(ln_stats, i, "out", c):
                     out = model(**c)["embedding"]
                 kept[i] = out
                 embs.append(out.detach())
@@ -357,19 +377,19 @@
                 if rand_states is not None:
                     rand_states[-1].restore()
                 _log_once(("gradcache-tail-oom",), "GradCache: a kept chunk ran out of memory; the rest of the step re-forwards")
-        with torch.no_grad():
+        with torch.no_grad(), _ln_stats_ctx(ln_stats, i, "out", c):
             embs.append(model(**c)["embedding"])
     return torch.cat(embs, dim=0)
 
 
-def accumulate_gradients(model, chunks, cache, rand_states=None, final: bool = False, skip=()):
+def accumulate_gradients(model, chunks, cache, rand_states=None, final: bool = False, skip=(), ln_stats=None):
     todo = [i for i in range(len(chunks)) if i not in skip]
     for i in todo:
         c, g = chunks[i], cache[i]
         state = rand_states[i] if rand_states is not None else RandContext(c, needed=False)
         if final and i == todo[-1] and hasattr(model, "arm_overlapped_reduce"):
             model.arm_overlapped_reduce()
-        with state:
+        with state, _ln_stats_ctx(ln_stats, i, "in", c):
             out = model(**c)["embedding"]
         out.backward(g.to(out.dtype))
 
@@ -636,9 +656,13 @@
                       f"{len(q_chunks)} + {len(d_chunks)}) keep their activations (no re-forward for them)")
         q_rnd, d_rnd = [], []
         q_kept, d_kept = {}, {}
+        q_stats, d_stats = _ln_stats_side(tower1, "q", pol), (_ln_stats_side(tower2, "d", pol) if was_training2 else None)
+        for st in (q_stats, d_stats):
+            if st is not None:
+                st[0].ln_stats_store.begin_step()
         try:
-            q_embs = get_chunked_embeddings(tower1, q_chunks, q_rnd, keep_tail=nq_keep, kept=q_kept)
-            d_embs = get_chunked_embeddings(tower2, d_chunks, d_rnd, keep_tail=nd_keep, kept=d_kept)
+            q_embs = get_chunked_embeddings(tower1, q_chunks, q_rnd, keep_tail=nq_keep, kept=q_kept, ln_stats=q_stats)
+            d_embs = get_chunked_embeddings(tower2, d_chunks, d_rnd, keep_tail=nd_keep, kept=d_kept, ln_stats=d_stats)
             q_cache, d_cache, loss = cache_loss(q_embs, d_embs, logit_scale, bidirectional=bidirectional, use_fp8=pol.use_fp8)
         except BaseException:
             _release_resident(tower1, list(q_kept.values()))
@@ -662,9 +686,9 @@
                 tower2.arm_overlapped_reduce()
             o.backward(d_grads[i].to(o.dtype))
         if re_q:
-            accumulate_gradients(tower1, q_chunks, q_grads, q_rnd, final=(not shared) or not re_d, skip=done_q)
+            accumulate_gradients(tower1, q_chunks, q_grads, q_rnd, final=(not shared) or not re_d, skip=done_q, ln_stats=q_stats)
         if re_d:
-            accumulate_gradients(tower2, d_chunks, d_grads, d_rnd, final=True, skip=done_d)
+            accumulate_gradients(tower2, d_chunks, d_grads, d_rnd, final=True, skip=done_d, ln_stats=d_stats)
     seen = set()
     for tw, active in ((tower1, was_training1), (tower2, was_training2)):
         if active and id(tw) not in seen and hasattr(tw, "sync_gradients"):
diff --git a/contrastors_amd/nomic_bert.py b/contrastors_amd/nomic_bert.py
--- a/contrastors_amd/nomic_bert.py
+++ b/contrastors_amd/nomic_bert.py
@@ -183,7 +183,7 @@
                 self.desc.checkpoint = int(self.checkpoint)
             elif name == "ckpt_keep":
                 self.desc.ckpt_keep = int(self.keep_layers)
-            elif name in ("drop_active", "drop_seed", "drop_offset", "n_keep", "n_patch_all"):
+            elif name in ("drop_active", "drop_seed", "drop_offset", "n_keep", "n_patch_all", "ln_stats_stride"):
                 setattr(self.desc, name, 0)
             else:
                 setattr(self.desc, name, t[name].data_ptr() if name in t else None)
@@ -197,6 +197,42 @@
         d, I, H = cfg.n_embd, cfg.n_inner, cfg.n_head
         extra = 2 * I + 4 * 2 if getattr(cfg, "norm_mlp", False) else 0
         return 2 * (3 * d + d + 3 * d + I + I) + 4 * (H + 4) + extra
+
+
+class LnStatsStore:
+
+    def __init__(self):
+        self._buf: Dict[object, torch.Tensor] = {}
+        self._sig: Dict[object, tuple] = {}
+
+    def begin_step(self):
+        self._sig.clear()
+
+    def invalidate(self, key):
+        self._sig.pop(key, None)
+
+    def valid(self, key) -> bool:
+        return key in self._sig
+
+    def for_write(self, key, n_layer: int, T: int, device, identity: tuple) -> torch.Tensor:
+        buf = self._buf.get(key)
+        if buf is None or buf.shape[0] != n_layer or buf.shape[2] < T or buf.device != device:
+            buf = self._buf[key] = torch.empty(n_layer, 4, _round_up(max(T, 1), 128), dtype=torch.float32, device=device)
+        self._sig[key] = identity
+        return buf
+
+    def for_read(self, key, identity: tuple) -> Optional[torch.Tensor]:
+        return self._buf[key] if self._sig.get(key) == identity else None
+
+    def nbytes(self) -> int:
+        return sum(b.numel() * 4 for b in self._buf.values())
+
+
+def _unbind_ln_stats(arena: _ChunkArena):
+    d = arena.desc
+    d.ln_stats_in = d.ln_stats_out = None
+    d.ln_stats_stride = 0
+    arena.ln_stats_buf = None
 
 
 _FULL_CACHE: Dict[tuple, tuple] = {}
@@ -318,6 +354,9 @@
         self._arena_nograd: Optional[_ChunkArena] = None
         self._arena_free: List[_ChunkArena] = []
         self._outstanding = 0
+        self.ln_stats_store = LnStatsStore()
+        self._ln_stats_req: Optional[tuple] = None
+        self.ln_stats_reforwards = 0
         self._overlap_armed = None
         self._ov_works = None
         self.gradient_checkpointing = False
@@ -694,6 +733,7 @@
     def release_arena(self, arena: _ChunkArena, used: bool = True):
         arena.emb_out = None
         arena.desc.layer_events = None
+        _unbind_ln_stats(arena)
         if used and getattr(arena, "probation", False) and self._plan_keep(arena):
             return
         self._arena_free.append(arena)
@@ -789,6 +829,7 @@
             out = torch.empty(vb.B, d, dtype=torch.float32, device=self.device_)
         arena = self._get_arena(vb.T, vb.B, save_for_backward)
         self._arm_dropout(arena)
+        self._bind_ln_stats(arena, vb, save_for_backward)
         self._desc.normalize = int(self.normalize_default if normalize is None else normalize)
         if vb.token_type_ids is None:
             rc = self.lib.cx_encoder_forward(C.byref(self._desc), C.byref(arena.desc), vb.input_ids.data_ptr(),
@@ -802,12 +843,48 @@
                                                    vb.cu_seqlens.data_ptr(), vb.B, vb.S, vb.T, vb.max_seqlen,
                                                    int(save_for_backward), out.data_ptr(), _C.cur_stream())
             _C.check(rc, "cx_encoder_forward_typed")
+        if not save_for_backward:
+            _unbind_ln_stats(arena)
         if save_for_backward:
             arena.emb_out = out
             arena.normalize = self._desc.normalize
             self._outstanding += 1
             return out, arena
         return out, None
+
+    @contextlib.contextmanager
+    def ln_stats_scope(self, key, mode: str, chunk_id: tuple):
+        prev, self._ln_stats_req = self._ln_stats_req, (key, mode, chunk_id)
+        try:
+            yield
+        finally:
+            self._ln_stats_req = prev
+
+    def _bind_ln_stats(self, arena: _ChunkArena, vb: VarlenBatch, save: bool):
+        d = arena.desc
+        _unbind_ln_stats(arena)
+        if self._ln_stats_req is None:
+            return
+        key, mode, chunk_id = self._ln_stats_req
+        store = self.ln_stats_store
+        eligible = not getattr(self.config, "prenorm", False) and not arena.checkpoint and not d.drop_active
+        identity = (chunk_id, vb.B, vb.S, vb.T)
+        buf = None
+        if mode == "out":
+            if save or not eligible:
+                store.invalidate(key)
+                return
+            buf = store.for_write(key, self.config.n_layer, vb.T, self.device_, identity)
+            d.ln_stats_out = buf.data_ptr()
+        elif mode == "in" and save and eligible:
+            buf = store.for_read(key, identity)
+            if buf is None:
+                return
+            d.ln_stats_in = buf.data_ptr()
+            self.ln_stats_reforwards += 1
+        if buf is not None:
+            d.ln_stats_stride = buf.shape[2]
+            arena.ln_stats_buf = buf
 
     def _check_token_types(self):
         if self.config.type_vocab_size != 2:
diff --git a/contrastors_amd/policy.py b/contrastors_amd/policy.py
--- a/contrastors_amd/policy.py
+++ b/contrastors_amd/policy.py
@@ -10,18 +10,22 @@
     chunk: Union[str, int] = "auto"
     resident: Union[str, bool] = "auto"
     use_fp8: bool = False
+    reforward_ln_stats: bool = True
 
     @classmethod
     def from_train_args(cls, ta) -> "GradCachePolicy":
         return cls(chunk=_parse_chunk(getattr(ta, "gradcache_chunk", "auto"), "train_args.gradcache_chunk"),
                    resident=_parse_resident(getattr(ta, "gradcache_resident", "auto"), "train_args.gradcache_resident"),
-                   use_fp8=bool(getattr(ta, "use_fp8", False)))
+                   use_fp8=bool(getattr(ta, "use_fp8", False)),
+                   reforward_ln_stats=bool(getattr(ta, "gradcache_ln_stats", True)))
 
     def with_env(self) -> "GradCachePolicy":
         c, r = os.environ.get("CX_GRADCACHE_CHUNK"), os.environ.get("CX_GRADCACHE_RESIDENT")
+        s = os.environ.get("CX_GRADCACHE_LN_STATS")
         return GradCachePolicy(chunk=self.chunk if c in (None, "") else _parse_chunk(c, "CX_GRADCACHE_CHUNK"),
                                resident=self.resident if r in (None, "") else _parse_resident(r, "CX_GRADCACHE_RESIDENT"),
-                               use_fp8=self.use_fp8)
+                               use_fp8=self.use_fp8,
+                               reforward_ln_stats=self.reforward_ln_stats if s in (None, "") else s.lower() not in ("0", "false", "no", "off"))
 
 
 def _parse_chunk(v, where: str):
diff --git a/include/contrastors_hip.h b/include/contrastors_hip.h
--- a/include/contrastors_hip.h
+++ b/include/contrastors_hip.h
@@ -110,6 +110,11 @@
 int cx_gemm_bf16_nt_residual(const uint16_t* X, const uint16_t* W, uint16_t* Out, const float* bias,
                              const uint16_t* Residual, int M, int N, int K, int ldx, int ldw, int ldo, int ldr,
                              void* stream);
+int cx_gemm_bf16_nt_residual_ln(const uint16_t* X, const uint16_t* W, uint16_t* Z, uint16_t* H, const float* bias,
+                                const uint16_t* Residual, const float* Mean, const float* Rstd, const float* Gamma,
+                                const float* Beta, int M, int N, int K, int ldx, int ldw, int ldz, int ldr, int ldh,
+                                void* stream);
+int cx_gemm_bf16_nt_residual_ln_min_tiles(void);
 int cx_gemm_bf16_nt_splitk(const uint16_t* X, const uint16_t* W, uint16_t* Out, const float* bias, const uint16_t* Residual,
                            float* ws, long ws_floats, int M, int N, int K, int ldx, int ldw, int ldo, int ldr, void* stream);
 int cx_gemm_bf16_swiglu(const uint16_t* X, const uint16_t* W, uint16_t* YG, uint16_t* Act, int M, int I, int K, int ldx,
@@ -341,6 +346,9 @@
     const int32_t* patch_inv;
     int n_keep;
     int n_patch_all;
+    const float* ln_stats_in;
+    float* ln_stats_out;
+    long ln_stats_stride;
 } CxChunkBuffers;
 
 int cx_encoder_forward(const CxEncoderDesc* enc, const CxChunkBuffers* buf, const int64_t* input_ids,
```

Result: no change. 4408 (median of 6 runs) (+0.9%).
